# BananaFalls/LDPC-NeuralNetwork-Decoder

Hardware: AMD Instinct MI355X
Metric: codewords/s at fixed SNR (BG2, 10 iters) (higher is better)
Workload: dtype f32

## Files before the change

### ldpc-neuralnetwork-decoder_amd/csrc/flood_fixed.hpp

```cpp
#pragma once
#include "flood_host.hpp"
#include "gen/fixed_codes.hpp"

namespace ldpc {
namespace {

constexpr bool reg_edges(int algo) { return algo == LDPC_ALGO_MINSUM; }

#ifndef LDPC_SLOW_REG_EDGES
#define LDPC_SLOW_REG_EDGES 16
#endif
#ifndef LDPC_SLOW_REG_EDGES_OFF
#define LDPC_SLOW_REG_EDGES_OFF 6
#endif
constexpr int kAllRegEdges = 1 << 20;
template <int ES, bool BAIL>
constexpr int reg_edge_cap() {
    return BAIL ? kAllRegEdges : (ES == LDPC_ES_OFF ? LDPC_SLOW_REG_EDGES_OFF : LDPC_SLOW_REG_EDGES);
}

#ifndef LDPC_ROT_EDGES
#define LDPC_ROT_EDGES (1 << 20)
#endif
#ifndef LDPC_SLOW_ROT_EDGES
#define LDPC_SLOW_ROT_EDGES (1 << 20)
#endif
#ifndef LDPC_SLOW_ROT_EDGES_OFF
#define LDPC_SLOW_ROT_EDGES_OFF 0
#endif
template <int ES, bool BAIL>
constexpr int rot_edge_cap() {
    return BAIL ? LDPC_ROT_EDGES : (ES == LDPC_ES_OFF ? LDPC_SLOW_ROT_EDGES_OFF : LDPC_SLOW_ROT_EDGES);
}

template <class G, int WV, int CAP, int RCAP, bool REG>
struct FxPlan {
    static constexpr int R0 = REG ? G::RE_CHK_PTR[WV] : G::CHK_PTR[WV];
    static constexpr int NR = (REG ? G::RE_CHK_PTR[WV + 1] : G::CHK_PTR[WV + 1]) - R0;
    static constexpr int NREG = !REG ? 0 : (G::RE_NREG[WV] < CAP ? G::RE_NREG[WV] : CAP);
    static constexpr int chk_row(int i) { return REG ? G::RE_CHK_ROWS[R0 + i] : G::CHK_ROWS[R0 + i]; }
    static constexpr int row_shift(int e) { return REG ? G::RE_ROW_SHIFT[e] : G::ROW_SHIFT[e]; }
    static constexpr int col_shift(int j) { return REG ? G::RE_COL_SHIFT[j] : G::COL_SHIFT[j]; }
    static constexpr int row_reg(int e) { return REG && G::RE_ROW_REG[e] < CAP ? G::RE_ROW_REG[e] : -1; }
    static constexpr int col_reg(int j) { return REG && G::RE_COL_REG[j] < CAP ? G::RE_COL_REG[j] : -1; }
    static constexpr int col_slot_edges(int w) {
        int n = 0;
        for (int i = G::VT_COL_PTR[w]; i < G::VT_COL_PTR[w + 1]; ++i)
            for (int j = G::COL_PTR[G::VT_COLS[i]]; j < G::COL_PTR[G::VT_COLS[i] + 1]; ++j)
                if (G::COL_SLOT[j] >= 0 && G::RE_COL_REG[j] < 0) ++n;
        return n;
    }
    static constexpr int rot_share() {
        if (!REG) return 0;
        int left = RCAP;
        for (int w = 0; w < G::W; ++w) {
            const int a = col_slot_edges(w), b = col_slot_edges(WV);
            if (a > b || (a == b && w < WV)) left -= G::RE_NROT[w];
        }
        return left < 0 ? 0 : (left < G::RE_NROT[WV] ? left : G::RE_NROT[WV]);
    }
    static constexpr int NROT = rot_share();
    static constexpr int row_rot(int e) { return REG && G::RE_ROW_ROT[e] < NROT ? G::RE_ROW_ROT[e] : -1; }
    static constexpr int col_rot(int j) { return REG && G::RE_COL_ROT[j] < NROT ? G::RE_COL_ROT[j] : -1; }
    static constexpr int C0 = G::VT_COL_PTR[WV], NC = G::VT_COL_PTR[WV + 1] - C0;
    static constexpr int T0 = G::VT_PTR[WV], NT = G::VT_PTR[WV + 1] - T0;
    static constexpr int col_index(int col) {
        for (int i = 0; i < NC; ++i)
            if (G::VT_COLS[C0 + i] == col) return i;
        return -1;
    }
    struct Tab {
        int nsh = 0, next = 0, maxdc = 1, maxdv = 1;
        int shv[64] = {};
        int shidx[64] = {};
        int ext_before[64] = {};
    };
    static constexpr int inv_shift(int s) { return (G::Z - s) % G::Z; }
    static constexpr Tab make() {
        Tab t{};
        for (int i = 0; i < 64; ++i) t.shidx[i] = -1;
        auto use = [&t](int s) {
            if (t.shidx[s] < 0) {
                t.shidx[s] = t.nsh;
                t.shv[t.nsh++] = s;
            }
        };
        for (int i = 0; i < NC; ++i) {
            const int c = G::VT_COLS[C0 + i];
            const int dv = G::COL_PTR[c + 1] - G::COL_PTR[c];
            if (dv > t.maxdv) t.maxdv = dv;
            for (int j = G::COL_PTR[c]; j < G::COL_PTR[c + 1]; ++j)
                if (col_reg(j) < 0 && col_rot(j) < 0) use(col_shift(j));
        }
        for (int i = 0; i < NR; ++i) {
            const int R = chk_row(i);
            t.ext_before[i] = t.next;
            const int dc = G::ROW_PTR[R + 1] - G::ROW_PTR[R];
            if (dc > t.maxdc) t.maxdc = dc;
            for (int e = G::ROW_PTR[R]; e < G::ROW_PTR[R + 1]; ++e) {
                if (G::ROW_SLOT[e] < 0)
                    ++t.next;
                else if (row_reg(e) < 0 && row_rot(e) < 0)
                    use(inv_shift(row_shift(e)));
            }
        }
        return t;
    }
    static constexpr Tab T = make();
    static constexpr int ext_index(int i, int e) {
        const int R = chk_row(i);
        int x = T.ext_before[i];
        for (int q = 0; q < e; ++q)
            if (G::ROW_SLOT[G::ROW_PTR[R] + q] < 0) ++x;
        return x;
    }
};

constexpr int kVarPipe = 24;

#ifndef LDPC_DIRECT_DC
#define LDPC_DIRECT_DC 6
#endif
constexpr int kDirectDc = LDPC_DIRECT_DC;
static_assert(kDirectDc >= 0 && kDirectDc <= 6, "direct_row is written out for degrees 2 .. 6");

__device__ __forceinline__ uint32_t xor3(uint32_t a, uint32_t b, uint32_t c) { return __builtin_amdgcn_bitop3_b32(a, b, c, 0x96); }

template <int DC, int E, int CAP>
__device__ __forceinline__ float direct_row(const float (&v)[CAP], const float (&pr)[3], float als, float alv, uint32_t sgn) {
    static_assert(DC >= 2 && DC <= 6 && E < DC && DC <= CAP, "direct form: degrees 2 .. 6");
    constexpr int A = E == 0 ? 1 : 0, B = E <= 1 ? 2 : 1, Cc = E <= 2 ? 3 : 2;
    auto bits = [&](int e) { return __float_as_uint(v[e]); };
    if constexpr (DC == 2) {
        return __uint_as_float(__builtin_amdgcn_bitop3_b32(__float_as_uint(alv * fabsf(v[A])), bits(A), sgn, 0x78));
    } else if constexpr (DC == 3) {
        const float m = vmin(fabsf(v[A]), fabsf(v[B]));
        return __uint_as_float(__builtin_amdgcn_bitop3_b32(__float_as_uint(alv * m), bits(A) ^ bits(B), sgn, 0x78));
    } else if constexpr (DC == 4) {
        const float m = vmin(vmin(fabsf(v[A]), fabsf(v[B])), fabsf(v[Cc]));
        return __uint_as_float(__builtin_amdgcn_bitop3_b32(__float_as_uint(alv * m), xor3(bits(A), bits(B), bits(Cc)), sgn, 0x78));
    } else {
        constexpr int PE = E / 2;
        float m;
        if constexpr (DC == 5 && E == 4)
            m = vmin(pr[0], pr[1]);
        else if constexpr (DC == 5)
            m = vmin(vmin(fabsf(v[E ^ 1]), pr[1 - PE]), fabsf(v[4]));
        else
            m = vmin(vmin(fabsf(v[E ^ 1]), pr[(PE + 1) % 3]), pr[(PE + 2) % 3]);
        return __uint_as_float(__builtin_amdgcn_bitop3_b32(__float_as_uint(als * m), bits(E), sgn, 0x78));
    }
}

constexpr int kOutAny = 2;
template <class G, int OUT>
struct DecOut {
    static_assert(OUT == LDPC_OUT_U8 || OUT == LDPC_OUT_F32 || OUT == kOutAny, "one form per output type");
    static_assert(G::N % G::Z == 0 && (G::Z & (G::Z - 1)) == 0, "rotated(): row | position");
    char *base;
    uint32_t row;
    uint32_t own;
    uint32_t kb;
    uint32_t any;
    bool valid;
    __device__ __forceinline__ uint32_t size() const {
        if constexpr (OUT == kOutAny)
            return any;
        else
            return OUT == LDPC_OUT_F32 ? 4u : 1u;
    }
    __device__ __forceinline__ DecOut(const Ctx &C, const Lane &L) {
        any = C.out_dtype == LDPC_OUT_F32 ? 4u : 1u;
        base = static_cast<char *>(C.bits) + (int64_t)L.group * (64 / G::Z) * G::N * size();
        row = (uint32_t)L.f * (G::N * size());
        kb = (uint32_t)L.k * size();
        own = row + kb;
        valid = L.valid;
    }
    __device__ __forceinline__ void put(uint32_t off, int bit, int &errs) const {
        if (valid) {
            if (size() == 4u)
                *reinterpret_cast<float *>(base + off) = (float)bit;
            else
                *reinterpret_cast<uint8_t *>(base + off) = (uint8_t)bit;
        }
        errs += bit;
    }
    template <int COL>
    __device__ __forceinline__ void col(int bit, int &errs) const { put(own + COL * G::Z * size(), bit, errs); }
    template <int COL, int S>
    __device__ __forceinline__ void rotated(int bit, int &errs) const {
        put((row | ((kb + S * size()) & (G::Z * size() - 1))) + COL * G::Z * size(), bit, errs);
    }
};
struct NoOut {
    __device__ __forceinline__ NoOut(const Ctx &, const Lane &) {}
};
template <class G, int OUT>
using DecOutFor = std::conditional_t<OUT < 0, NoOut, DecOut<G, OUT>>;

template <class G, int ALGO, int WV, bool BAIL, int CAP, int RCAP, bool REG>
struct FixedBody {
    static_assert(!BAIL || ALGO == LDPC_ALGO_MINSUM, "only min-sum has a fast and an exact check update");
    static constexpr bool kBail = BAIL;
    static constexpr bool kPeel = true;
    using P = FxPlan<G, WV, CAP, RCAP, REG>;
    static constexpr int ZM4 = 4 * G::Z - 1;
    static constexpr int NEXT = P::T.next > 0 ? P::T.next : 1;
    static constexpr int NCOL = P::NC > 0 ? P::NC : 1;
    static constexpr int NSH = P::T.nsh > 0 ? P::T.nsh : 1;
    static constexpr int MAXDC = P::T.maxdc, MAXDV = P::T.maxdv;
    static constexpr int NRG = P::NREG > 0 ? P::NREG : 1;
    static constexpr int NRT = P::NROT > 0 ? P::NROT : 1;
    float ext[NEXT];
    float cllr[NCOL];
    uint32_t rot[NSH];
    float msg[NRG];
    float rmsg[NRT];


    template <int S>
    __device__ __forceinline__ float to_var_lane(float c2v) const { return seg_rotate<G::Z, S>(c2v); }
    template <int S>
    __device__ __forceinline__ float to_chk_lane(float v2c) const { return seg_rotate<G::Z, P::inv_shift(S)>(v2c); }

    __device__ __forceinline__ void init(Ctx &C, const Lane &L) {
        bool nan = false;
        sfor<P::NR>([&](auto i) {
            constexpr int I = decltype(i)::value, R = P::chk_row(I);
            constexpr int P0 = G::ROW_PTR[R], DC = G::ROW_PTR[R + 1] - P0;
            sfor<DC>([&](auto e) {
                constexpr int E = decltype(e)::value;
                if constexpr (G::ROW_SLOT[P0 + E] < 0) {
                    constexpr int X = P::ext_index(I, E), COL = G::ROW_COL[P0 + E], S4 = 4 * P::row_shift(P0 + E);
                    ext[X] = L.llr_at(COL * 4 * G::Z + ((L.k4 + S4) & ZM4));
                    nan |= !(fabsf(ext[X]) < INFINITY);
                }
            });
        });
        sfor<P::T.nsh>([&](auto j) {
            constexpr int J = decltype(j)::value, SH = P::T.shv[J];
            const uint32_t base = (uint32_t)(uintptr_t)C.lds;
            if constexpr (SH == 0)
                rot[J] = opaque_vu(base + L.lane4);
            else
                rot[J] = opaque_vu(base + L.fz4 + ((L.k4 + (4 * G::Z - 4 * SH)) & ZM4));
        });
        addtid_begin(C.lds);
        sfor<P::NC>([&](auto i) {
            constexpr int I = decltype(i)::value, COL = G::VT_COLS[P::C0 + I];
            constexpr int P0 = G::COL_PTR[COL], DV = G::COL_PTR[COL + 1] - P0;
            cllr[I] = L.llr_at(COL * 4 * G::Z + L.k4);
            nan |= !(fabsf(cllr[I]) < INFINITY);
            sfor<DV>([&](auto jj) {
                constexpr int J = P0 + decltype(jj)::value;
                if constexpr (P::col_reg(J) >= 0)
                    msg[P::col_reg(J)] = cllr[I];
                else if constexpr (P::col_rot(J) >= 0)
                    rmsg[P::col_rot(J)] = to_chk_lane<P::col_shift(J)>(cllr[I]);
                else
                    lds_wr_tid<G::COL_SLOT[J] * 256>(cllr[I]);
            });
        });
        addtid_end();
        if (__any(nan) && L.lane == 0) *C.flag = 1;
    }

    template <int I>
    __device__ __forceinline__ void load_row(const Ctx &C, const Lane &L, float (&v)[MAXDC]) const {
        constexpr int R = P::chk_row(I), P0 = G::ROW_PTR[R], DC = G::ROW_PTR[R + 1] - P0;
        sfor<DC>([&](auto e) {
            constexpr int E = decltype(e)::value, SL = G::ROW_SLOT[P0 + E];
            if constexpr (P::row_reg(P0 + E) >= 0)
                v[E] = msg[P::row_reg(P0 + E)];
            else if constexpr (P::row_rot(P0 + E) >= 0)
                v[E] = rmsg[P::row_rot(P0 + E)];
            else if constexpr (SL >= 0)
                v[E] = lds_rd_abs<SL * 256>(rot[P::T.shidx[P::inv_shift(P::row_shift(P0 + E))]]);
            else
                v[E] = ext[P::ext_index(I, E)];
        });
    }

    template <int I, bool DEC, bool SLOW, int OUT>
    __device__ __forceinline__ void row(const Ctx &C, const Lane &L, const DecOutFor<G, OUT> &D, const float (&v)[MAXDC], int &errs, float ninf, float pinf, uint32_t sgn, float alv) {
        constexpr int R = P::chk_row(I), P0 = G::ROW_PTR[R], DC = G::ROW_PTR[R + 1] - P0;
        auto needed = [](int e) constexpr { return DEC || G::ROW_SLOT[P0 + e] >= 0; };
        auto emit = [&](auto e, float o) {
            constexpr int E = decltype(e)::value, SL = G::ROW_SLOT[P0 + E];
            if constexpr (P::row_reg(P0 + E) >= 0) {
                msg[P::row_reg(P0 + E)] = o;
            } else if constexpr (P::row_rot(P0 + E) >= 0) {
                rmsg[P::row_rot(P0 + E)] = to_var_lane<P::row_shift(P0 + E)>(o);
            } else if constexpr (SL >= 0) {
                lds_wr_tid<SL * 256>(o);
            } else if constexpr (DEC) {
                constexpr int COL = G::ROW_COL[P0 + E], S = P::row_shift(P0 + E);
                const int bit = v[E] + o < 0.0f;
                if constexpr (OUT >= 0) D.template rotated<COL, S>(bit, errs);
                if (C.ballots) ext_ballot(C, L, COL, 4 * S, bit);
            }
        };
        if constexpr (ALGO == LDPC_ALGO_MINSUM && !SLOW && DC >= 2 && DC <= kDirectDc) {
            float pr[3] = {};
            float als = alv;
            if constexpr (DC >= 5) {
                sfor<DC / 2>([&](auto j) {
                    constexpr int J = decltype(j)::value;
                    pr[J] = vmin(fabsf(v[2 * J]), fabsf(v[2 * J + 1]));
                });
                uint32_t par = xor3(__float_as_uint(v[0]), __float_as_uint(v[1]), __float_as_uint(v[2]));
                if constexpr (DC == 5)
                    par = xor3(par, __float_as_uint(v[3]), __float_as_uint(v[4]));
                else
                    par = xor3(par, __float_as_uint(v[3]), __float_as_uint(v[4])) ^ __float_as_uint(v[5]);
                als = __uint_as_float(__builtin_amdgcn_bitop3_b32(__float_as_uint(alv), par, sgn, 0x78));
            }
            sfor<DC>([&](auto e) {
                constexpr int E = decltype(e)::value;
                if constexpr (needed(E)) emit(e, direct_row<DC, E>(v, pr, als, alv, sgn));
            });
        } else if constexpr (ALGO == LDPC_ALGO_MINSUM) {
            float m1 = fabsf(v[0]), m2 = pinf;
            two_smallest<DC>(v, m1, m2, ninf);
            if (!SLOW) {
                const uint32_t par = sign_parity_n<DC>(v) & sgn;
                const uint32_t s1 = __float_as_uint(alv * m1) ^ par, s2 = __float_as_uint(alv * m2) ^ par;
                uint64_t mk[DC];
                uint32_t sel[DC];
                sfor<DC + 3>([&](auto q) {
                    constexpr int Q = decltype(q)::value;
                    if constexpr (Q < DC && needed(Q)) mk[Q] = cmp_eq_abs(v[Q], m1);
                    if constexpr (Q >= 3 && needed(Q - 3)) sel[Q - 3] = cndmask(s1, s2, mk[Q - 3]);
                });
                sfor<DC>([&](auto e) {
                    constexpr int E = decltype(e)::value;
                    if constexpr (needed(E))
                        emit(e, __uint_as_float(__builtin_amdgcn_bitop3_b32(sel[E], __float_as_uint(v[E]), sgn, 0x78)));
                });
            } else {
                MinSumStats st;
                sfor<DC>([&](auto e) { st.add(decltype(e)::value, v[decltype(e)::value]); });
                sfor<DC>([&](auto e) { emit(e, st.c2v(decltype(e)::value, v[decltype(e)::value], C.alpha)); });
            }
        } else {
            float acc[DC];
            float Pp = 1.0f;
            sfor<DC>([&](auto jj) {
                constexpr int J = decltype(jj)::value;
                const float t = tanh_half(v[J]);
                sfor<J>([&](auto e) { acc[decltype(e)::value] = acc[decltype(e)::value] * t; });
                acc[J] = Pp;
                Pp = Pp * t;
            });
            sfor<DC>([&](auto e) { emit(e, two_atanh(acc[decltype(e)::value])); });
        }
    }

    template <bool DEC, bool DIRECT>
    __device__ __forceinline__ void check(const Ctx &C, const Lane &L, int &errs) {
        static_assert(DEC || !DIRECT, "stores need decisions");
        if constexpr (ALGO == LDPC_ALGO_MINSUM && !BAIL) {
            if (__builtin_amdgcn_readfirstlane(*C.flag) != 0) {
                rows<DEC, true, (DIRECT ? kOutAny : -1)>(C, L, errs);
                return;
            }
        }
        if constexpr (!DIRECT)
            rows<DEC, false, -1>(C, L, errs);
        else if (C.out_dtype == LDPC_OUT_F32)
            rows<DEC, false, LDPC_OUT_F32>(C, L, errs);
        else
            rows<DEC, false, LDPC_OUT_U8>(C, L, errs);
    }

    template <bool DEC, bool SLOW, int OUT>
    __device__ __forceinline__ void rows(const Ctx &C, const Lane &L, int &errs) {
        float va[MAXDC], vb[MAXDC];
        const DecOutFor<G, OUT> D(C, L);
        addtid_begin(C.lds);
        const float ninf = opaque_sf(-INFINITY), pinf = opaque_sf(INFINITY);
        const uint32_t sgn = opaque_vu(0x80000000u);
        const float alv = opaque_vf(C.alpha);
        load_row<0>(C, L, va);
        sfor<P::NR>([&](auto i) {
            constexpr int I = decltype(i)::value;
            if constexpr (I % 2 == 0) {
                if constexpr (I + 1 < P::NR) load_row<I + 1>(C, L, vb);
                row<I, DEC, SLOW, OUT>(C, L, D, va, errs, ninf, pinf, sgn, alv);
            } else {
                if constexpr (I + 1 < P::NR) load_row<I + 1>(C, L, va);
                row<I, DEC, SLOW, OUT>(C, L, D, vb, errs, ninf, pinf, sgn, alv);
            }
        });
        addtid_end();
    }

    template <int TK>
    struct Task {
        static constexpr int X = P::T0 + TK;
        static constexpr int CA = G::VT_A[X], CB = G::VT_B[X];
        static constexpr int PA = G::COL_PTR[CA], DA = G::COL_PTR[CA + 1] - PA;
        static constexpr int PB = CB >= 0 ? G::COL_PTR[CB] : 0, DB = CB >= 0 ? G::COL_PTR[CB + 1] - PB : 0;
        static_assert(DB <= DA, "pair tasks: A is the longer column");
        static constexpr int IA = P::col_index(CA), IB = CB >= 0 ? P::col_index(CB) : 0;
        static constexpr int NMSG = DA + DB;
    };
    struct TaskIn {
        f32x2 cp[MAXDV];
        float cs[MAXDV];
    };

    template <int X>
    __device__ __forceinline__ float c2v_in() const {
        if constexpr (P::col_reg(X) >= 0)
            return msg[P::col_reg(X)];
        else if constexpr (P::col_rot(X) >= 0)
            return rmsg[P::col_rot(X)];
        else
            return lds_rd_abs<G::COL_SLOT[X] * 256>(rot[P::T.shidx[P::col_shift(X)]]);
    }
    template <int X>
    __device__ __forceinline__ void v2c_out(float o) {
        if constexpr (P::col_reg(X) >= 0)
            msg[P::col_reg(X)] = o;
        else if constexpr (P::col_rot(X) >= 0)
            rmsg[P::col_rot(X)] = to_chk_lane<P::col_shift(X)>(o);
        else
            lds_wr_tid<G::COL_SLOT[X] * 256>(o);
    }

    template <int TK>
    __device__ __forceinline__ void load_task(const Ctx &C, TaskIn &in) const {
        using K = Task<TK>;
        sfor<K::DA>([&](auto jj) {
            constexpr int J = decltype(jj)::value;
            if constexpr (J < K::DB) {
                in.cp[J].x = c2v_in<K::PA + J>();
                in.cp[J].y = c2v_in<K::PB + J>();
            } else {
                in.cs[J] = c2v_in<K::PA + J>();
            }
        });
    }

    template <int TK, bool DEC, bool WRITE, int OUT>
    __device__ __forceinline__ void task(const Ctx &C, const Lane &L, const DecOutFor<G, OUT> &D, const TaskIn &in, int &errs, bool &bad) {
        using K = Task<TK>;
        constexpr int DA = K::DA, DB = K::DB;
        f32x2 P2;
        float PA = cllr[K::IA];
        if constexpr (DB > 0) {
            P2.x = cllr[K::IA];
            P2.y = cllr[K::IB];
        }
        f32x2 acc2[DB > 0 ? DB : 1];
        float accA[DA];
        sfor<DA>([&](auto jj) {
            constexpr int J = decltype(jj)::value;
            if constexpr (J < DB) {
                sfor<J>([&](auto e) {
                    constexpr int E = decltype(e)::value;
                    acc2[E] = acc2[E] + in.cp[J];
                });
                acc2[J] = P2;
                P2 = P2 + in.cp[J];
                if constexpr (J == DB - 1) PA = P2.x;
            } else {
                sfor<J>([&](auto e) {
                    constexpr int E = decltype(e)::value;
                    if constexpr (E < DB)
                        acc2[E].x = acc2[E].x + in.cs[J];
                    else
                        accA[E] = accA[E] + in.cs[J];
                });
                accA[J] = PA;
                PA = PA + in.cs[J];
            }
        });
        if constexpr (WRITE) {
            sfor<DA>([&](auto e) {
                constexpr int E = decltype(e)::value;
                if constexpr (E < DB) {
                    v2c_out<K::PA + E>(acc2[E].x);
                    v2c_out<K::PB + E>(acc2[E].y);
                } else {
                    v2c_out<K::PA + E>(accA[E]);
                }
            });
        }
        auto decide = [&](auto col, float app) {
            constexpr int COL = decltype(col)::value;
            const int bit = app < 0.0f;
            if constexpr (OUT >= 0) D.template col<COL>(bit, errs);
            if (C.ballots) var_ballot(C, L, COL, bit);
        };
        if constexpr (ALGO == LDPC_ALGO_MINSUM) bad |= !(fabsf(PA) < INFINITY);
        if constexpr (DEC) decide(ic<K::CA>{}, PA);
        if constexpr (DB > 0) {
            if constexpr (ALGO == LDPC_ALGO_MINSUM) bad |= !(fabsf(P2.y) < INFINITY);
            if constexpr (DEC) decide(ic<K::CB>{}, P2.y);
        }
    }

    template <bool DEC, bool WRITE, bool DIRECT>
    __device__ __forceinline__ void var(const Ctx &C, const Lane &L, int &errs) {
        static_assert(DEC || !DIRECT, "stores need decisions");
        if constexpr (!DIRECT)
            var_as<DEC, WRITE, -1>(C, L, errs);
        else if (C.out_dtype == LDPC_OUT_F32)
            var_as<DEC, WRITE, LDPC_OUT_F32>(C, L, errs);
        else
            var_as<DEC, WRITE, LDPC_OUT_U8>(C, L, errs);
    }
    template <bool DEC, bool WRITE, int OUT>
    __device__ __forceinline__ void var_as(const Ctx &C, const Lane &L, int &errs) {
        bool bad = false;
        if constexpr (P::NT > 0) {
            const DecOutFor<G, OUT> D(C, L);
            TaskIn ta, tb;
            if constexpr (WRITE) addtid_begin(C.lds);
            load_task<0>(C, ta);
            sfor<P::NT>([&](auto i) {
                constexpr int I = decltype(i)::value;
                constexpr bool more = I + 1 < P::NT;
                constexpr bool ahead = more && Task<I>::NMSG + Task<(more ? I + 1 : I)>::NMSG <= kVarPipe;
                if constexpr (I % 2 == 0) {
                    if constexpr (ahead) load_task<I + 1>(C, tb);
                    task<I, DEC, WRITE, OUT>(C, L, D, ta, errs, bad);
                    if constexpr (more && !ahead) load_task<(more ? I + 1 : I)>(C, tb);
                } else {
                    if constexpr (ahead) load_task<I + 1>(C, ta);
                    task<I, DEC, WRITE, OUT>(C, L, D, tb, errs, bad);
                    if constexpr (more && !ahead) load_task<(more ? I + 1 : I)>(C, ta);
                }
            });
            if constexpr (WRITE) addtid_end();
        }
        if constexpr (ALGO == LDPC_ALGO_MINSUM) {
            if (__any(bad) && L.lane == 0) *C.flag = 1;
        }
    }

    __device__ __forceinline__ int parity(const Ctx &C, const Lane &L) const {
        int inv = 0;
        int f = L.f, k = L.k;
        asm volatile("" : "+v"(f), "+v"(k));
        sfor<P::NR>([&](auto i) {
            constexpr int R = P::chk_row(decltype(i)::value);
            constexpr int P0 = G::ROW_PTR[R], DC = G::ROW_PTR[R + 1] - P0;
            int p = 0;
            sfor<DC>([&](auto e) {
                constexpr int E = decltype(e)::value;
                constexpr int COL = G::ROW_COL[P0 + E], S = P::row_shift(P0 + E);
                p ^= (int)(C.words[COL] >> (f * G::Z + ((k + S) & (G::Z - 1))));
            });
            inv |= p;
        });
        return inv & 1;
    }
};

template <class G, class F>
__device__ __forceinline__ void fx_by_wave(int wave, F &&f) {
    static_assert(G::W == 4, "fixed schedules are generated for 4 waves");
    switch (wave) {
        case 0: f(ic<0>{}); break;
        case 1: f(ic<1>{}); break;
        case 2: f(ic<2>{}); break;
        default: f(ic<3>{}); break;
    }
}

}

template <class G, int ALGO, int ES, bool BAIL = false>
__global__ __launch_bounds__(256, ES == LDPC_ES_OFF ? 4 : 3) void flood_fixed_kernel(FloodTables T, const float *__restrict__ llr,
                                                          int64_t B, int max_iter, float alpha, int out_dtype,
                                                          void *__restrict__ bits, Outs O, EsWs W, uint32_t *redo) {
    static_assert(!BAIL || ES == LDPC_ES_OFF || ES == LDPC_ES_FRAME, "the batch-stop passes share state across workgroups");
    extern __shared__ __attribute__((aligned(16))) char lds[];
#ifdef LDPC_TIMELINE
    const uint64_t t_in = tl_now();
#endif
    FloodTables Tc = T;
    Tc.Z = G::Z, Tc.FG = 64 / G::Z, Tc.Mb = G::Mb, Tc.Nb = G::Nb, Tc.N = G::N, Tc.nslots = G::NSLOTS, Tc.W = G::W;
    static_assert(G::Z < 64 && 64 % G::Z == 0, "rep1 below: a 1 at the bottom of every Z-bit segment");
    Tc.rep1 = ~0ull / ((1ull << G::Z) - 1ull);
    const Lane L = make_lane(Tc, llr, B);
    Ctx C;
    init_ctx(C, Tc, lds, alpha, out_dtype, bits);
    if constexpr (BAIL) C.redo = redo;
    fx_by_wave<G>(__builtin_amdgcn_readfirstlane((int)threadIdx.x >> 6), [&](auto wv) {
        FixedBody<G, ALGO, decltype(wv)::value, BAIL, reg_edge_cap<ES, BAIL>(), rot_edge_cap<ES, BAIL>(), reg_edges(ALGO)> body;
        flood_drive<ES>(body, C, L, B, max_iter, O, W);
#ifdef LDPC_TIMELINE
        if constexpr (ES == LDPC_ES_OFF) tl_bracket(O.timeline, decltype(wv)::value, t_in);
#endif
    });
}

template <int ALGO>
int launch_fixed(const FloodCall &c, int es, size_t lds, const Outs &O, const EsWs &W, uint32_t *redo) {
    auto pick = [&](auto code) -> const void * {
        using G = decltype(code);
        if constexpr (ALGO == LDPC_ALGO_MINSUM) {
            if (redo && es == LDPC_ES_OFF) return reinterpret_cast<const void *>(flood_fixed_kernel<G, ALGO, LDPC_ES_OFF, true>);
            if (redo && es == LDPC_ES_FRAME) return reinterpret_cast<const void *>(flood_fixed_kernel<G, ALGO, LDPC_ES_FRAME, true>);
        }
        if (redo) return nullptr;
        switch (es) {
            case LDPC_ES_OFF: return reinterpret_cast<const void *>(flood_fixed_kernel<G, ALGO, LDPC_ES_OFF>);
            case LDPC_ES_FRAME: return reinterpret_cast<const void *>(flood_fixed_kernel<G, ALGO, LDPC_ES_FRAME>);
            case LDPC_ES_BATCH: return reinterpret_cast<const void *>(flood_fixed_kernel<G, ALGO, LDPC_ES_BATCH>);
            case ES_P1: return reinterpret_cast<const void *>(flood_fixed_kernel<G, ALGO, ES_P1>);
            case ES_P2: return reinterpret_cast<const void *>(flood_fixed_kernel<G, ALGO, ES_P2>);
            default: return nullptr;
        }
    };
    const int id = c.g->fixed_id;
    const void *kern = id == 1 ? pick(fixed::BG2_Z4{}) : (id == 2 ? pick(fixed::BG2_Z32{}) : nullptr);
    if (!kern) return fail(LDPC_EINVAL, "no fixed kernel for this code / stopping mode");
    LDPC_HIP(hipFuncSetAttribute(kern, hipFuncAttributeMaxDynamicSharedMemorySize, (int)lds));
    FloodCall a = c;
    FloodTables t = c.g->ft;
    Outs o = O;
    EsWs w = W;
    void *args[] = {&t, &a.llr, &a.B, &a.max_iter, &a.alpha, &a.out_dtype, &a.bits, &o, &w, &redo};
    const int64_t nwg = (c.B + c.g->FG - 1) / c.g->FG;
    LDPC_HIP(hipLaunchKernel(kern, dim3((unsigned)nwg), dim3(64 * c.g->ft.W), args, lds, c.s));
    return LDPC_OK;
}

}
```

### ldpc-neuralnetwork-decoder_amd/csrc/gen/fixed_codes.hpp

```cpp
#pragma once

namespace ldpc {
namespace fixed {

struct BG2_Z4 {
    static constexpr int Z = 4, Mb = 42, Nb = 52, N = 208, NSLOTS = 159, W = 4;
    static constexpr int NBLOCKS = 197;
    static constexpr int BLK_ROW[197] = {0, 0, 0, 0, 0, 0, 0, 0, 1, 1, 1, 1, 1, 1, 1, 1, 1, 1, 2, 2, 2, 2, 2, 2, 2, 2, 3, 3, 3, 3, 3, 3, 3, 3, 3, 3, 4, 4, 4, 4, 5, 5, 5, 5, 5, 5, 6, 6, 6, 6, 6, 6, 7, 7, 7, 7, 7, 7, 8, 8, 8, 8, 9, 9, 9, 9, 9, 10, 10, 10, 10, 10, 11, 11, 11, 11, 11, 12, 12, 12, 12, 13, 13, 13, 13, 13, 14, 14, 14, 14, 14, 15, 15, 15, 15, 16, 16, 16, 16, 16, 17, 17, 17, 17, 17, 18, 18, 18, 18, 19, 19, 19, 19, 20, 20, 20, 20, 21, 21, 21, 21, 22, 22, 22, 23, 23, 23, 23, 24, 24, 24, 24, 25, 25, 25, 26, 26, 26, 26, 26, 27, 27, 27, 28, 28, 28, 28, 29, 29, 29, 30, 30, 30, 30, 30, 31, 31, 31, 32, 32, 32, 32, 33, 33, 33, 33, 34, 34, 34, 34, 35, 35, 35, 35, 36, 36, 36, 36, 37, 37, 37, 38, 38, 38, 38, 39, 39, 39, 39, 40, 40, 40, 40, 41, 41, 41, 41};
    static constexpr int BLK_COL[197] = {0, 1, 2, 3, 6, 9, 10, 11, 0, 3, 4, 5, 6, 7, 8, 9, 11, 12, 0, 1, 3, 4, 8, 10, 12, 13, 1, 2, 4, 5, 6, 7, 8, 9, 10, 13, 0, 1, 11, 14, 0, 1, 5, 7, 11, 15, 0, 5, 7, 9, 11, 16, 1, 5, 7, 11, 13, 17, 0, 1, 12, 18, 1, 8, 10, 11, 19, 0, 1, 6, 7, 20, 0, 7, 9, 13, 21, 1, 3, 11, 22, 0, 1, 8, 13, 23, 1, 6, 11, 13, 24, 0, 10, 11, 25, 1, 9, 11, 12, 26, 1, 5, 11, 12, 27, 0, 6, 7, 28, 0, 1, 10, 29, 1, 4, 11, 30, 0, 8, 13, 31, 1, 2, 32, 0, 3, 5, 33, 1, 2, 9, 34, 0, 5, 35, 2, 7, 12, 13, 36, 0, 6, 37, 1, 2, 5, 38, 0, 4, 39, 2, 5, 7, 9, 40, 1, 13, 41, 0, 5, 12, 42, 2, 7, 10, 43, 0, 12, 13, 44, 1, 5, 11, 45, 0, 2, 7, 46, 10, 13, 47, 1, 5, 11, 48, 0, 7, 12, 49, 2, 10, 13, 50, 1, 5, 11, 51};
    static constexpr int BLK_SHIFT[197] = {1, 1, 0, 2, 1, 1, 0, 0, 3, 2, 1, 1, 2, 0, 0, 0, 0, 0, 1, 2, 0, 0, 0, 1, 0, 0, 0, 2, 2, 0, 1, 2, 2, 0, 0, 0, 3, 2, 3, 0, 3, 1, 2, 3, 3, 0, 3, 0, 1, 0, 2, 0, 1, 3, 0, 3, 0, 0, 2, 2, 2, 0, 3, 1, 1, 3, 0, 3, 1, 0, 1, 0, 3, 0, 2, 0, 0, 3, 3, 2, 0, 3, 2, 2, 2, 0, 3, 1, 3, 0, 0, 3, 3, 1, 0, 3, 2, 0, 2, 0, 2, 0, 2, 0, 0, 0, 2, 2, 0, 3, 0, 1, 0, 2, 1, 1, 0, 0, 2, 2, 0, 2, 3, 0, 3, 3, 2, 0, 2, 3, 0, 0, 0, 0, 0, 1, 3, 0, 2, 0, 0, 3, 0, 2, 1, 3, 0, 2, 0, 0, 3, 0, 1, 0, 0, 2, 1, 0, 2, 0, 2, 0, 0, 0, 3, 0, 3, 1, 0, 0, 1, 0, 3, 0, 0, 2, 2, 0, 3, 3, 0, 3, 2, 2, 0, 3, 0, 2, 0, 0, 3, 0, 0, 1, 1, 2, 0};
    static constexpr int ROW_PTR[43] = {0, 8, 18, 26, 36, 40, 46, 52, 58, 62, 67, 72, 77, 81, 86, 91, 95, 100, 105, 109, 113, 117, 121, 124, 128, 132, 135, 140, 143, 147, 150, 155, 158, 162, 166, 170, 174, 178, 181, 185, 189, 193, 197};
    static constexpr int ROW_SLOT[197] = {0, 1, 2, 3, 4, 5, 6, 7, 8, 9, 10, 11, 12, 13, 14, 15, 16, 17, 18, 19, 20, 21, 22, 23, 24, 25, 26, 27, 28, 29, 30, 31, 32, 33, 34, 35, 36, 37, 38, -1, 39, 40, 41, 42, 43, -1, 44, 45, 46, 47, 48, -1, 49, 50, 51, 52, 53, -1, 54, 55, 56, -1, 57, 58, 59, 60, -1, 61, 62, 63, 64, -1, 65, 66, 67, 68, -1, 69, 70, 71, -1, 72, 73, 74, 75, -1, 76, 77, 78, 79, -1, 80, 81, 82, -1, 83, 84, 85, 86, -1, 87, 88, 89, 90, -1, 91, 92, 93, -1, 94, 95, 96, -1, 97, 98, 99, -1, 100, 101, 102, -1, 103, 104, -1, 105, 106, 107, -1, 108, 109, 110, -1, 111, 112, -1, 113, 114, 115, 116, -1, 117, 118, -1, 119, 120, 121, -1, 122, 123, -1, 124, 125, 126, 127, -1, 128, 129, -1, 130, 131, 132, -1, 133, 134, 135, -1, 136, 137, 138, -1, 139, 140, 141, -1, 142, 143, 144, -1, 145, 146, -1, 147, 148, 149, -1, 150, 151, 152, -1, 153, 154, 155, -1, 156, 157, 158, -1};
    static constexpr int ROW_COL[197] = {0, 1, 2, 3, 6, 9, 10, 11, 0, 3, 4, 5, 6, 7, 8, 9, 11, 12, 0, 1, 3, 4, 8, 10, 12, 13, 1, 2, 4, 5, 6, 7, 8, 9, 10, 13, 0, 1, 11, 14, 0, 1, 5, 7, 11, 15, 0, 5, 7, 9, 11, 16, 1, 5, 7, 11, 13, 17, 0, 1, 12, 18, 1, 8, 10, 11, 19, 0, 1, 6, 7, 20, 0, 7, 9, 13, 21, 1, 3, 11, 22, 0, 1, 8, 13, 23, 1, 6, 11, 13, 24, 0, 10, 11, 25, 1, 9, 11, 12, 26, 1, 5, 11, 12, 27, 0, 6, 7, 28, 0, 1, 10, 29, 1, 4, 11, 30, 0, 8, 13, 31, 1, 2, 32, 0, 3, 5, 33, 1, 2, 9, 34, 0, 5, 35, 2, 7, 12, 13, 36, 0, 6, 37, 1, 2, 5, 38, 0, 4, 39, 2, 5, 7, 9, 40, 1, 13, 41, 0, 5, 12, 42, 2, 7, 10, 43, 0, 12, 13, 44, 1, 5, 11, 45, 0, 2, 7, 46, 10, 13, 47, 1, 5, 11, 48, 0, 7, 12, 49, 2, 10, 13, 50, 1, 5, 11, 51};
    static constexpr int ROW_SHIFT[197] = {1, 1, 0, 2, 1, 1, 0, 0, 3, 2, 1, 1, 2, 0, 0, 0, 0, 0, 1, 2, 0, 0, 0, 1, 0, 0, 0, 2, 2, 0, 1, 2, 2, 0, 0, 0, 3, 2, 3, 0, 3, 1, 2, 3, 3, 0, 3, 0, 1, 0, 2, 0, 1, 3, 0, 3, 0, 0, 2, 2, 2, 0, 3, 1, 1, 3, 0, 3, 1, 0, 1, 0, 3, 0, 2, 0, 0, 3, 3, 2, 0, 3, 2, 2, 2, 0, 3, 1, 3, 0, 0, 3, 3, 1, 0, 3, 2, 0, 2, 0, 2, 0, 2, 0, 0, 0, 2, 2, 0, 3, 0, 1, 0, 2, 1, 1, 0, 0, 2, 2, 0, 2, 3, 0, 3, 3, 2, 0, 2, 3, 0, 0, 0, 0, 0, 1, 3, 0, 2, 0, 0, 3, 0, 2, 1, 3, 0, 2, 0, 0, 3, 0, 1, 0, 0, 2, 1, 0, 2, 0, 2, 0, 0, 0, 3, 0, 3, 1, 0, 0, 1, 0, 3, 0, 0, 2, 2, 0, 3, 3, 0, 3, 2, 2, 0, 3, 0, 2, 0, 0, 3, 0, 0, 1, 1, 2, 0};
    static constexpr int COL_PTR[53] = {0, 22, 45, 55, 60, 65, 79, 86, 99, 105, 113, 122, 138, 147, 159, 160, 161, 162, 163, 164, 165, 166, 167, 168, 169, 170, 171, 172, 173, 174, 175, 176, 177, 178, 179, 180, 181, 182, 183, 184, 185, 186, 187, 188, 189, 190, 191, 192, 193, 194, 195, 196, 197};
    static constexpr int COL_SLOT[197] = {0, 8, 18, 36, 39, 44, 54, 61, 65, 72, 80, 91, 94, 100, 105, 111, 117, 122, 130, 136, 142, 150, 1, 19, 26, 37, 40, 49, 55, 57, 62, 69, 73, 76, 83, 87, 95, 97, 103, 108, 119, 128, 139, 147, 156, 2, 27, 104, 109, 113, 120, 124, 133, 143, 153, 3, 9, 20, 70, 106, 10, 21, 28, 98, 123, 11, 29, 41, 45, 50, 88, 107, 112, 121, 125, 131, 140, 148, 157, 4, 12, 30, 63, 77, 92, 118, 13, 31, 42, 46, 51, 64, 66, 93, 114, 126, 134, 144, 151, 14, 22, 32, 58, 74, 101, 5, 15, 33, 47, 67, 84, 110, 127, 6, 23, 34, 59, 81, 96, 135, 145, 154, 7, 16, 38, 43, 48, 52, 60, 71, 78, 82, 85, 89, 99, 141, 149, 158, 17, 24, 56, 86, 90, 115, 132, 137, 152, 25, 35, 53, 68, 75, 79, 102, 116, 129, 138, 146, 155, -1, -1, -1, -1, -1, -1, -1, -1, -1, -1, -1, -1, -1, -1, -1, -1, -1, -1, -1, -1, -1, -1, -1, -1, -1, -1, -1, -1, -1, -1, -1, -1, -1, -1, -1, -1, -1, -1};
    static constexpr int COL_SHIFT[197] = {1, 3, 1, 3, 3, 3, 2, 3, 3, 3, 3, 0, 3, 0, 3, 0, 0, 2, 2, 3, 0, 3, 1, 2, 0, 2, 1, 1, 2, 3, 1, 3, 2, 3, 3, 2, 0, 2, 2, 2, 2, 2, 1, 3, 1, 0, 2, 3, 3, 1, 1, 3, 0, 2, 0, 2, 2, 0, 3, 3, 1, 0, 2, 1, 0, 1, 0, 2, 0, 3, 0, 2, 0, 3, 0, 0, 0, 2, 1, 1, 2, 1, 0, 1, 2, 3, 0, 2, 3, 1, 0, 1, 0, 2, 3, 1, 0, 2, 0, 0, 0, 2, 1, 2, 2, 1, 0, 0, 0, 2, 2, 0, 0, 0, 1, 0, 1, 3, 1, 3, 3, 3, 0, 0, 3, 3, 2, 3, 3, 2, 3, 1, 0, 2, 1, 3, 2, 2, 0, 0, 2, 2, 0, 0, 2, 1, 2, 0, 0, 0, 0, 2, 0, 2, 2, 1, 0, 3, 0, 0, 0, 0, 0, 0, 0, 0, 0, 0, 0, 0, 0, 0, 0, 0, 0, 0, 0, 0, 0, 0, 0, 0, 0, 0, 0, 0, 0, 0, 0, 0, 0, 0, 0, 0, 0, 0, 0};
    static constexpr int CHK_PTR[5] = {0, 10, 21, 32, 42};
    static constexpr int CHK_ROWS[42] = {3, 9, 12, 13, 15, 20, 26, 28, 35, 40, 0, 4, 5, 10, 16, 18, 22, 23, 29, 33, 38, 2, 6, 8, 11, 17, 19, 24, 25, 31, 34, 39, 1, 7, 14, 21, 27, 30, 32, 36, 37, 41};
    static constexpr int VT_COL_PTR[5] = {0, 3, 7, 10, 14};
    static constexpr int VT_COLS[14] = {0, 4, 12, 3, 5, 9, 11, 1, 6, 8, 2, 7, 10, 13};
    static constexpr int VT_PTR[5] = {0, 3, 6, 8, 10};
    static constexpr int VT_A[10] = {0, 4, 12, 3, 9, 11, 1, 6, 2, 7};
    static constexpr int VT_B[10] = {-1, -1, -1, -1, -1, 5, -1, 8, 10, 13};
    static constexpr int BW_PTR[5] = {0, 13, 26, 39, 52};
    static constexpr int BW_COLS[52] = {0, 4, 8, 12, 16, 20, 24, 28, 32, 36, 40, 44, 48, 1, 5, 9, 13, 17, 21, 25, 29, 33, 37, 41, 45, 49, 2, 6, 10, 14, 18, 22, 26, 30, 34, 38, 42, 46, 50, 3, 7, 11, 15, 19, 23, 27, 31, 35, 39, 43, 47, 51};
    static constexpr int RE_CAP = 16;
    static constexpr int RE_RHO[42] = {3, 0, 0, 0, 1, 1, 0, 1, 2, 3, 0, 0, 1, 2, 1, 1, 2, 2, 0, 0, 2, 0, 2, 1, 2, 0, 1, 1, 1, 0, 0, 2, 2, 0, 1, 0, 2, 1, 2, 1, 0, 3};
    static constexpr int RE_ROW_SHIFT[197] = {0, 0, 3, 1, 0, 0, 3, 3, 3, 2, 1, 1, 2, 0, 0, 0, 0, 0, 1, 2, 0, 0, 0, 1, 0, 0, 0, 2, 2, 0, 1, 2, 2, 0, 0, 0, 0, 3, 0, 1, 0, 2, 3, 0, 0, 1, 3, 0, 1, 0, 2, 0, 2, 0, 1, 0, 1, 1, 0, 0, 0, 2, 2, 0, 0, 2, 3, 3, 1, 0, 1, 0, 3, 0, 2, 0, 0, 0, 0, 3, 1, 1, 0, 0, 0, 2, 0, 2, 0, 1, 1, 0, 0, 2, 1, 1, 0, 2, 0, 2, 0, 2, 0, 2, 2, 0, 2, 2, 0, 3, 0, 1, 0, 0, 3, 3, 2, 0, 2, 2, 0, 0, 1, 2, 0, 0, 3, 1, 0, 1, 2, 2, 0, 0, 0, 2, 0, 1, 3, 1, 1, 0, 1, 3, 2, 0, 1, 2, 0, 0, 3, 0, 1, 0, 0, 0, 3, 2, 0, 2, 0, 2, 0, 0, 3, 0, 0, 2, 1, 1, 1, 0, 3, 0, 2, 0, 0, 2, 0, 0, 1, 1, 0, 0, 2, 0, 1, 3, 1, 0, 3, 0, 0, 0, 0, 1, 3};
    static constexpr int RE_COL_SHIFT[197] = {0, 3, 1, 0, 0, 3, 0, 3, 3, 1, 0, 0, 3, 0, 0, 0, 1, 2, 0, 0, 2, 0, 0, 2, 0, 3, 2, 2, 0, 2, 1, 0, 0, 0, 1, 0, 0, 0, 0, 0, 3, 0, 1, 1, 0, 3, 2, 1, 1, 2, 2, 3, 0, 0, 0, 1, 2, 0, 0, 0, 1, 0, 2, 3, 0, 1, 0, 3, 0, 0, 2, 3, 0, 0, 0, 2, 0, 0, 0, 0, 2, 1, 0, 2, 2, 0, 0, 2, 0, 1, 1, 1, 0, 2, 0, 1, 0, 0, 1, 0, 0, 2, 0, 0, 2, 0, 0, 0, 0, 2, 0, 2, 0, 3, 1, 0, 0, 0, 1, 3, 0, 3, 3, 0, 0, 0, 2, 0, 2, 3, 0, 2, 2, 0, 3, 3, 0, 1, 0, 0, 0, 0, 2, 1, 0, 2, 3, 0, 0, 1, 0, 0, 1, 2, 3, 3, 1, 0, 0, 1, 1, 0, 1, 2, 3, 0, 0, 1, 2, 1, 1, 2, 2, 0, 0, 2, 0, 2, 1, 2, 0, 1, 1, 1, 0, 0, 2, 2, 0, 1, 0, 2, 1, 2, 1, 0, 3};
    static constexpr int RE_ROW_REG[197] = {-1, 0, -1, -1, 1, -1, -1, -1, -1, -1, -1, -1, -1, -1, -1, 0, 1, -1, -1, -1, -1, 0, -1, -1, 1, -1, -1, -1, -1, -1, -1, -1, -1, -1, 0, 1, 2, -1, -1, -1, -1, -1, -1, 2, -1, -1, -1, 2, -1, 3, -1, -1, -1, 4, -1, 5, -1, -1, 3, -1, 4, -1, -1, -1, 3, -1, -1, -1, -1, 2, -1, -1, -1, 4, -1, 5, -1, 3, -1, -1, -1, -1, 4, 5, -1, -1, -1, -1, 6, -1, -1, 5, -1, -1, -1, -1, -1, -1, 6, -1, 6, -1, -1, -1, -1, 7, -1, -1, -1, -1, 7, -1, -1, 8, -1, -1, -1, 8, -1, -1, -1, 9, -1, -1, 9, -1, -1, -1, 10, -1, -1, -1, -1, 7, -1, -1, 6, -1, -1, -1, -1, 11, -1, -1, -1, 8, -1, -1, 10, -1, -1, 9, -1, 10, -1, 12, -1, -1, 11, -1, 12, -1, 7, 8, -1, -1, 13, -1, -1, -1, -1, 11, -1, -1, -1, 9, 10, -1, 11, 12, -1, -1, 12, 13, -1, 14, -1, -1, -1, 13, -1, 14, -1, 13, -1, -1, -1};
    static constexpr int RE_COL_REG[197] = {-1, -1, -1, 2, -1, -1, 3, -1, -1, -1, 5, 7, -1, 8, 9, -1, -1, -1, 11, 13, -1, 14, 0, -1, -1, -1, -1, -1, -1, -1, -1, 3, 4, -1, -1, 6, 7, 8, 9, 10, -1, 12, -1, -1, 13, -1, -1, -1, -1, -1, -1, -1, 7, 9, 13, -1, -1, -1, -1, -1, -1, 0, -1, -1, 10, -1, -1, -1, 2, 4, -1, -1, 7, 8, 9, -1, 11, 12, -1, 1, -1, -1, 2, -1, -1, 11, -1, -1, 2, -1, -1, -1, 4, -1, 6, -1, 8, 10, -1, -1, -1, -1, -1, 5, -1, -1, 0, -1, 3, -1, -1, -1, 10, -1, -1, 0, 3, -1, -1, -1, 11, -1, -1, 1, -1, -1, -1, 5, -1, -1, 6, -1, -1, -1, -1, -1, 13, -1, -1, 1, 4, 6, -1, -1, 12, -1, -1, -1, 1, -1, 5, -1, -1, -1, -1, -1, -1, 12, 14, -1, -1, -1, -1, -1, -1, -1, -1, -1, -1, -1, -1, -1, -1, -1, -1, -1, -1, -1, -1, -1, -1, -1, -1, -1, -1, -1, -1, -1, -1, -1, -1, -1, -1, -1, -1, -1, -1};
    static constexpr int RE_NREG[4] = {15, 14, 14, 15};
    static constexpr int RE_CHK_PTR[5] = {0, 12, 21, 33, 42};
    static constexpr int RE_CHK_ROWS[42] = {2, 4, 8, 15, 16, 18, 21, 23, 29, 32, 34, 39, 1, 6, 7, 14, 25, 28, 30, 35, 38, 0, 10, 12, 13, 17, 19, 20, 22, 24, 27, 31, 41, 3, 5, 9, 11, 26, 33, 36, 37, 40};
    static constexpr int RE_ROW_ROT[197] = {-1, -1, -1, -1, -1, -1, -1, -1, -1, 0, -1, 1, -1, -1, -1, -1, -1, -1, 0, -1, -1, -1, -1, -1, -1, -1, -1, 0, -1, -1, -1, 1, -1, -1, -1, -1, -1, -1, -1, -1, -1, -1, -1, -1, -1, -1, -1, -1, -1, -1, 2, -1, -1, -1, -1, -1, -1, -1, -1, -1, -1, -1, -1, -1, -1, -1, -1, -1, 0, -1, -1, -1, -1, -1, -1, -1, -1, -1, -1, -1, -1, -1, -1, -1, -1, -1, -1, -1, -1, -1, -1, -1, -1, -1, -1, -1, -1, -1, -1, -1, -1, -1, -1, -1, -1, -1, -1, -1, -1, -1, -1, -1, -1, -1, -1, -1, -1, -1, -1, -1, -1, -1, -1, -1, -1, -1, -1, -1, -1, -1, -1, -1, -1, -1, -1, 2, -1, -1, 3, -1, -1, -1, -1, -1, -1, -1, -1, 1, -1, -1, -1, -1, -1, -1, -1, -1, -1, -1, -1, -1, -1, -1, -1, -1, 4, -1, -1, 2, -1, -1, -1, -1, 3, -1, -1, -1, -1, -1, -1, -1, -1, -1, -1, -1, -1, -1, -1, 3, -1, -1, 5, -1, -1, -1, -1, -1, -1};
    static constexpr int RE_COL_ROT[197] = {-1, -1, 0, -1, -1, -1, -1, -1, -1, -1, -1, -1, -1, -1, -1, -1, -1, 1, -1, -1, -1, -1, -1, -1, -1, -1, -1, -1, -1, -1, 0, -1, -1, -1, -1, -1, -1, -1, -1, -1, -1, -1, -1, -1, -1, -1, 0, -1, -1, 2, -1, -1, -1, -1, -1, -1, 0, -1, -1, -1, -1, -1, -1, -1, -1, 1, -1, -1, -1, -1, -1, -1, -1, -1, -1, -1, -1, -1, -1, -1, -1, -1, -1, -1, -1, -1, -1, 1, -1, -1, -1, -1, -1, -1, -1, -1, -1, -1, -1, -1, -1, -1, -1, -1, -1, -1, -1, -1, -1, -1, -1, -1, -1, -1, -1, -1, -1, -1, -1, 4, -1, 5, -1, -1, -1, -1, 2, -1, -1, -1, -1, -1, -1, -1, -1, 3, -1, -1, -1, -1, -1, -1, -1, -1, -1, 2, 3, -1, -1, -1, -1, -1, -1, -1, 3, -1, -1, -1, -1, -1, -1, -1, -1, -1, -1, -1, -1, -1, -1, -1, -1, -1, -1, -1, -1, -1, -1, -1, -1, -1, -1, -1, -1, -1, -1, -1, -1, -1, -1, -1, -1, -1, -1, -1, -1, -1, -1};
    static constexpr int RE_NROT[4] = {4, 4, 1, 6};
};

struct BG2_Z32 {
    static constexpr int Z = 32, Mb = 42, Nb = 52, N = 1664, NSLOTS = 159, W = 4;
    static constexpr int NBLOCKS = 197;
    static constexpr int BLK_ROW[197] = {0, 0, 0, 0, 0, 0, 0, 0, 1, 1, 1, 1, 1, 1, 1, 1, 1, 1, 2, 2, 2, 2, 2, 2, 2, 2, 3, 3, 3, 3, 3, 3, 3, 3, 3, 3, 4, 4, 4, 4, 5, 5, 5, 5, 5, 5, 6, 6, 6, 6, 6, 6, 7, 7, 7, 7, 7, 7, 8, 8, 8, 8, 9, 9, 9, 9, 9, 10, 10, 10, 10, 10, 11, 11, 11, 11, 11, 12, 12, 12, 12, 13, 13, 13, 13, 13, 14, 14, 14, 14, 14, 15, 15, 15, 15, 16, 16, 16, 16, 16, 17, 17, 17, 17, 17, 18, 18, 18, 18, 19, 19, 19, 19, 20, 20, 20, 20, 21, 21, 21, 21, 22, 22, 22, 23, 23, 23, 23, 24, 24, 24, 24, 25, 25, 25, 26, 26, 26, 26, 26, 27, 27, 27, 28, 28, 28, 28, 29, 29, 29, 30, 30, 30, 30, 30, 31, 31, 31, 32, 32, 32, 32, 33, 33, 33, 33, 34, 34, 34, 34, 35, 35, 35, 35, 36, 36, 36, 36, 37, 37, 37, 38, 38, 38, 38, 39, 39, 39, 39, 40, 40, 40, 40, 41, 41, 41, 41};
    static constexpr int BLK_COL[197] = {0, 1, 2, 3, 6, 9, 10, 11, 0, 3, 4, 5, 6, 7, 8, 9, 11, 12, 0, 1, 3, 4, 8, 10, 12, 13, 1, 2, 4, 5, 6, 7, 8, 9, 10, 13, 0, 1, 11, 14, 0, 1, 5, 7, 11, 15, 0, 5, 7, 9, 11, 16, 1, 5, 7, 11, 13, 17, 0, 1, 12, 18, 1, 8, 10, 11, 19, 0, 1, 6, 7, 20, 0, 7, 9, 13, 21, 1, 3, 11, 22, 0, 1, 8, 13, 23, 1, 6, 11, 13, 24, 0, 10, 11, 25, 1, 9, 11, 12, 26, 1, 5, 11, 12, 27, 0, 6, 7, 28, 0, 1, 10, 29, 1, 4, 11, 30, 0, 8, 13, 31, 1, 2, 32, 0, 3, 5, 33, 1, 2, 9, 34, 0, 5, 35, 2, 7, 12, 13, 36, 0, 6, 37, 1, 2, 5, 38, 0, 4, 39, 2, 5, 7, 9, 40, 1, 13, 41, 0, 5, 12, 42, 2, 7, 10, 43, 0, 12, 13, 44, 1, 5, 11, 45, 0, 2, 7, 46, 10, 13, 47, 1, 5, 11, 48, 0, 7, 12, 49, 2, 10, 13, 50, 1, 5, 11, 51};
    static constexpr int BLK_SHIFT[197] = {9, 21, 12, 26, 29, 13, 0, 0, 7, 6, 29, 29, 2, 28, 0, 28, 0, 0, 17, 18, 12, 20, 16, 1, 0, 0, 8, 26, 30, 8, 17, 22, 18, 0, 0, 0, 19, 22, 7, 0, 7, 9, 2, 31, 7, 0, 27, 4, 13, 28, 30, 0, 1, 19, 12, 3, 20, 0, 14, 30, 6, 0, 11, 13, 29, 23, 0, 11, 25, 0, 21, 0, 11, 12, 18, 24, 0, 31, 15, 14, 0, 19, 2, 6, 30, 0, 19, 17, 3, 8, 0, 19, 15, 21, 0, 11, 14, 8, 18, 0, 30, 28, 18, 0, 0, 28, 2, 18, 0, 23, 20, 25, 0, 26, 9, 29, 0, 12, 10, 18, 0, 30, 31, 0, 23, 11, 14, 0, 14, 11, 8, 0, 4, 28, 0, 29, 15, 0, 26, 0, 8, 23, 0, 2, 5, 7, 0, 18, 28, 0, 7, 16, 9, 20, 0, 10, 1, 0, 18, 12, 6, 0, 4, 4, 11, 0, 19, 21, 4, 0, 25, 8, 31, 0, 12, 6, 26, 0, 27, 23, 0, 31, 2, 6, 0, 15, 12, 2, 0, 0, 11, 24, 0, 1, 5, 22, 0};
    static constexpr int ROW_PTR[43] = {0, 8, 18, 26, 36, 40, 46, 52, 58, 62, 67, 72, 77, 81, 86, 91, 95, 100, 105, 109, 113, 117, 121, 124, 128, 132, 135, 140, 143, 147, 150, 155, 158, 162, 166, 170, 174, 178, 181, 185, 189, 193, 197};
    static constexpr int ROW_SLOT[197] = {0, 1, 2, 3, 4, 5, 6, 7, 8, 9, 10, 11, 12, 13, 14, 15, 16, 17, 18, 19, 20, 21, 22, 23, 24, 25, 26, 27, 28, 29, 30, 31, 32, 33, 34, 35, 36, 37, 38, -1, 39, 40, 41, 42, 43, -1, 44, 45, 46, 47, 48, -1, 49, 50, 51, 52, 53, -1, 54, 55, 56, -1, 57, 58, 59, 60, -1, 61, 62, 63, 64, -1, 65, 66, 67, 68, -1, 69, 70, 71, -1, 72, 73, 74, 75, -1, 76, 77, 78, 79, -1, 80, 81, 82, -1, 83, 84, 85, 86, -1, 87, 88, 89, 90, -1, 91, 92, 93, -1, 94, 95, 96, -1, 97, 98, 99, -1, 100, 101, 102, -1, 103, 104, -1, 105, 106, 107, -1, 108, 109, 110, -1, 111, 112, -1, 113, 114, 115, 116, -1, 117, 118, -1, 119, 120, 121, -1, 122, 123, -1, 124, 125, 126, 127, -1, 128, 129, -1, 130, 131, 132, -1, 133, 134, 135, -1, 136, 137, 138, -1, 139, 140, 141, -1, 142, 143, 144, -1, 145, 146, -1, 147, 148, 149, -1, 150, 151, 152, -1, 153, 154, 155, -1, 156, 157, 158, -1};
    static constexpr int ROW_COL[197] = {0, 1, 2, 3, 6, 9, 10, 11, 0, 3, 4, 5, 6, 7, 8, 9, 11, 12, 0, 1, 3, 4, 8, 10, 12, 13, 1, 2, 4, 5, 6, 7, 8, 9, 10, 13, 0, 1, 11, 14, 0, 1, 5, 7, 11, 15, 0, 5, 7, 9, 11, 16, 1, 5, 7, 11, 13, 17, 0, 1, 12, 18, 1, 8, 10, 11, 19, 0, 1, 6, 7, 20, 0, 7, 9, 13, 21, 1, 3, 11, 22, 0, 1, 8, 13, 23, 1, 6, 11, 13, 24, 0, 10, 11, 25, 1, 9, 11, 12, 26, 1, 5, 11, 12, 27, 0, 6, 7, 28, 0, 1, 10, 29, 1, 4, 11, 30, 0, 8, 13, 31, 1, 2, 32, 0, 3, 5, 33, 1, 2, 9, 34, 0, 5, 35, 2, 7, 12, 13, 36, 0, 6, 37, 1, 2, 5, 38, 0, 4, 39, 2, 5, 7, 9, 40, 1, 13, 41, 0, 5, 12, 42, 2, 7, 10, 43, 0, 12, 13, 44, 1, 5, 11, 45, 0, 2, 7, 46, 10, 13, 47, 1, 5, 11, 48, 0, 7, 12, 49, 2, 10, 13, 50, 1, 5, 11, 51};
    static constexpr int ROW_SHIFT[197] = {9, 21, 12, 26, 29, 13, 0, 0, 7, 6, 29, 29, 2, 28, 0, 28, 0, 0, 17, 18, 12, 20, 16, 1, 0, 0, 8, 26, 30, 8, 17, 22, 18, 0, 0, 0, 19, 22, 7, 0, 7, 9, 2, 31, 7, 0, 27, 4, 13, 28, 30, 0, 1, 19, 12, 3, 20, 0, 14, 30, 6, 0, 11, 13, 29, 23, 0, 11, 25, 0, 21, 0, 11, 12, 18, 24, 0, 31, 15, 14, 0, 19, 2, 6, 30, 0, 19, 17, 3, 8, 0, 19, 15, 21, 0, 11, 14, 8, 18, 0, 30, 28, 18, 0, 0, 28, 2, 18, 0, 23, 20, 25, 0, 26, 9, 29, 0, 12, 10, 18, 0, 30, 31, 0, 23, 11, 14, 0, 14, 11, 8, 0, 4, 28, 0, 29, 15, 0, 26, 0, 8, 23, 0, 2, 5, 7, 0, 18, 28, 0, 7, 16, 9, 20, 0, 10, 1, 0, 18, 12, 6, 0, 4, 4, 11, 0, 19, 21, 4, 0, 25, 8, 31, 0, 12, 6, 26, 0, 27, 23, 0, 31, 2, 6, 0, 15, 12, 2, 0, 0, 11, 24, 0, 1, 5, 22, 0};
    static constexpr int COL_PTR[53] = {0, 22, 45, 55, 60, 65, 79, 86, 99, 105, 113, 122, 138, 147, 159, 160, 161, 162, 163, 164, 165, 166, 167, 168, 169, 170, 171, 172, 173, 174, 175, 176, 177, 178, 179, 180, 181, 182, 183, 184, 185, 186, 187, 188, 189, 190, 191, 192, 193, 194, 195, 196, 197};
    static constexpr int COL_SLOT[197] = {0, 8, 18, 36, 39, 44, 54, 61, 65, 72, 80, 91, 94, 100, 105, 111, 117, 122, 130, 136, 142, 150, 1, 19, 26, 37, 40, 49, 55, 57, 62, 69, 73, 76, 83, 87, 95, 97, 103, 108, 119, 128, 139, 147, 156, 2, 27, 104, 109, 113, 120, 124, 133, 143, 153, 3, 9, 20, 70, 106, 10, 21, 28, 98, 123, 11, 29, 41, 45, 50, 88, 107, 112, 121, 125, 131, 140, 148, 157, 4, 12, 30, 63, 77, 92, 118, 13, 31, 42, 46, 51, 64, 66, 93, 114, 126, 134, 144, 151, 14, 22, 32, 58, 74, 101, 5, 15, 33, 47, 67, 84, 110, 127, 6, 23, 34, 59, 81, 96, 135, 145, 154, 7, 16, 38, 43, 48, 52, 60, 71, 78, 82, 85, 89, 99, 141, 149, 158, 17, 24, 56, 86, 90, 115, 132, 137, 152, 25, 35, 53, 68, 75, 79, 102, 116, 129, 138, 146, 155, -1, -1, -1, -1, -1, -1, -1, -1, -1, -1, -1, -1, -1, -1, -1, -1, -1, -1, -1, -1, -1, -1, -1, -1, -1, -1, -1, -1, -1, -1, -1, -1, -1, -1, -1, -1, -1, -1};
    static constexpr int COL_SHIFT[197] = {9, 7, 17, 19, 7, 27, 14, 11, 11, 19, 19, 28, 23, 12, 23, 4, 8, 18, 18, 19, 12, 15, 21, 18, 8, 22, 9, 1, 30, 11, 25, 31, 2, 19, 11, 30, 20, 26, 30, 14, 2, 10, 25, 31, 1, 12, 26, 31, 11, 29, 5, 7, 4, 6, 0, 26, 6, 12, 15, 11, 29, 20, 30, 9, 28, 29, 8, 2, 4, 19, 28, 14, 28, 7, 16, 12, 8, 2, 5, 29, 2, 17, 0, 17, 2, 23, 28, 22, 31, 13, 12, 21, 12, 18, 15, 9, 4, 26, 12, 0, 16, 18, 13, 6, 10, 13, 28, 0, 28, 18, 14, 8, 20, 0, 1, 0, 29, 15, 25, 11, 27, 11, 0, 0, 7, 7, 30, 3, 23, 14, 3, 21, 8, 18, 29, 31, 6, 22, 0, 0, 6, 18, 0, 0, 6, 21, 2, 0, 0, 20, 24, 30, 8, 18, 26, 1, 4, 23, 24, 0, 0, 0, 0, 0, 0, 0, 0, 0, 0, 0, 0, 0, 0, 0, 0, 0, 0, 0, 0, 0, 0, 0, 0, 0, 0, 0, 0, 0, 0, 0, 0, 0, 0, 0, 0, 0, 0};
    static constexpr int CHK_PTR[5] = {0, 10, 21, 32, 42};
    static constexpr int CHK_ROWS[42] = {3, 9, 12, 13, 15, 20, 26, 28, 35, 40, 0, 4, 5, 10, 16, 18, 22, 23, 29, 33, 38, 2, 6, 8, 11, 17, 19, 24, 25, 31, 34, 39, 1, 7, 14, 21, 27, 30, 32, 36, 37, 41};
    static constexpr int VT_COL_PTR[5] = {0, 3, 7, 10, 14};
    static constexpr int VT_COLS[14] = {0, 4, 12, 3, 5, 9, 11, 1, 6, 8, 2, 7, 10, 13};
    static constexpr int VT_PTR[5] = {0, 3, 6, 8, 10};
    static constexpr int VT_A[10] = {0, 4, 12, 3, 9, 11, 1, 6, 2, 7};
    static constexpr int VT_B[10] = {-1, -1, -1, -1, -1, 5, -1, 8, 10, 13};
    static constexpr int BW_PTR[5] = {0, 13, 26, 39, 52};
    static constexpr int BW_COLS[52] = {0, 4, 8, 12, 16, 20, 24, 28, 32, 36, 40, 44, 48, 1, 5, 9, 13, 17, 21, 25, 29, 33, 37, 41, 45, 49, 2, 6, 10, 14, 18, 22, 26, 30, 34, 38, 42, 46, 50, 3, 7, 11, 15, 19, 23, 27, 31, 35, 39, 43, 47, 51};
    static constexpr int RE_CAP = 16;
    static constexpr int RE_RHO[42] = {6, 0, 14, 0, 13, 1, 19, 31, 2, 21, 11, 14, 1, 2, 13, 11, 18, 0, 4, 9, 3, 20, 2, 21, 18, 4, 0, 24, 30, 4, 12, 22, 20, 28, 11, 7, 20, 5, 30, 20, 0, 10};
    static constexpr int RE_ROW_SHIFT[197] = {15, 27, 18, 0, 3, 19, 6, 6, 7, 6, 29, 29, 2, 28, 0, 28, 0, 0, 31, 0, 26, 2, 30, 15, 14, 14, 8, 26, 30, 8, 17, 22, 18, 0, 0, 0, 0, 3, 20, 13, 8, 10, 3, 0, 8, 1, 14, 23, 0, 15, 17, 19, 0, 18, 11, 2, 19, 31, 16, 0, 8, 2, 0, 2, 18, 12, 21, 22, 4, 11, 0, 11, 25, 26, 0, 6, 14, 0, 16, 15, 1, 21, 4, 8, 0, 2, 0, 30, 16, 21, 13, 30, 26, 0, 11, 29, 0, 26, 4, 18, 30, 28, 18, 0, 0, 0, 6, 22, 4, 0, 29, 2, 9, 29, 12, 0, 3, 0, 30, 6, 20, 0, 1, 2, 12, 0, 3, 21, 0, 29, 26, 18, 8, 0, 4, 29, 15, 0, 26, 0, 0, 15, 24, 0, 3, 5, 30, 22, 0, 4, 19, 28, 21, 0, 12, 0, 23, 22, 6, 0, 26, 20, 0, 0, 7, 28, 30, 0, 15, 11, 0, 15, 6, 7, 0, 26, 14, 20, 0, 28, 5, 29, 0, 4, 30, 3, 0, 22, 20, 0, 11, 24, 0, 11, 15, 0, 10};
    static constexpr int RE_COL_SHIFT[197] = {15, 7, 31, 0, 8, 14, 16, 22, 25, 21, 30, 0, 0, 0, 12, 8, 0, 22, 6, 30, 0, 3, 27, 0, 8, 3, 10, 0, 0, 0, 4, 0, 4, 0, 29, 30, 29, 29, 0, 0, 0, 0, 0, 29, 11, 18, 26, 1, 29, 29, 3, 19, 0, 26, 0, 0, 6, 26, 16, 0, 29, 2, 30, 12, 0, 29, 8, 3, 23, 18, 28, 3, 0, 5, 28, 0, 15, 0, 15, 3, 2, 17, 11, 30, 6, 15, 28, 22, 0, 0, 11, 0, 26, 22, 15, 21, 0, 14, 0, 0, 30, 18, 2, 8, 30, 19, 28, 0, 15, 0, 0, 26, 0, 6, 15, 0, 18, 26, 2, 7, 0, 11, 6, 0, 20, 8, 17, 2, 12, 15, 16, 0, 26, 18, 0, 6, 4, 0, 0, 14, 8, 4, 0, 0, 26, 0, 22, 14, 0, 19, 6, 0, 21, 6, 26, 23, 15, 28, 24, 13, 1, 19, 31, 2, 21, 11, 14, 1, 2, 13, 11, 18, 0, 4, 9, 3, 20, 2, 21, 18, 4, 0, 24, 30, 4, 12, 22, 20, 28, 11, 7, 20, 5, 30, 20, 0, 10};
    static constexpr int RE_ROW_REG[197] = {-1, -1, -1, 0, -1, -1, -1, -1, -1, -1, -1, -1, -1, -1, -1, -1, -1, 0, -1, 0, -1, -1, -1, -1, -1, -1, -1, -1, -1, -1, -1, -1, -1, -1, 0, 1, 1, -1, -1, -1, -1, -1, -1, 2, -1, -1, -1, -1, 3, -1, -1, -1, 1, -1, -1, -1, -1, -1, -1, 2, -1, -1, 3, -1, -1, -1, -1, -1, -1, -1, 4, -1, -1, -1, 1, -1, -1, 4, -1, -1, -1, -1, -1, -1, 5, -1, 5, -1, -1, -1, -1, -1, -1, 2, -1, -1, 3, -1, -1, -1, -1, -1, -1, 2, -1, 3, -1, -1, -1, 4, -1, -1, -1, -1, -1, 4, -1, 5, -1, -1, -1, 6, -1, -1, -1, 5, -1, -1, 7, -1, -1, -1, -1, 6, -1, -1, -1, 6, -1, -1, 7, -1, -1, 8, -1, -1, -1, -1, 8, -1, -1, -1, -1, 7, -1, 9, -1, -1, -1, 8, -1, -1, 6, 7, -1, -1, -1, 9, -1, -1, 10, -1, -1, -1, 10, -1, -1, -1, 8, -1, -1, -1, 9, -1, -1, -1, 9, -1, -1, 10, -1, -1, -1, -1, -1, 10, -1};
    static constexpr int RE_COL_REG[197] = {-1, -1, -1, 1, -1, -1, -1, -1, -1, -1, -1, 3, 4, 5, -1, -1, 7, -1, -1, -1, 10, -1, -1, 0, -1, -1, -1, 1, 2, 3, -1, 4, -1, 5, -1, -1, -1, -1, 6, 7, 8, 9, 10, -1, -1, -1, -1, -1, -1, -1, -1, -1, 6, -1, 10, 0, -1, -1, -1, 5, -1, -1, -1, -1, 8, -1, -1, -1, -1, -1, -1, -1, 6, -1, -1, 8, -1, 9, -1, -1, -1, -1, -1, -1, -1, -1, -1, -1, 2, 3, -1, 4, -1, -1, -1, -1, 7, -1, 9, -1, -1, -1, -1, -1, -1, -1, -1, -1, -1, 1, 3, -1, 7, -1, -1, 0, -1, -1, -1, -1, 8, -1, -1, -1, -1, -1, -1, -1, -1, -1, -1, 2, -1, -1, 4, -1, -1, 10, 0, -1, -1, -1, 2, 6, -1, 9, -1, -1, 1, -1, -1, 5, -1, -1, -1, -1, -1, -1, -1, -1, -1, -1, -1, -1, -1, -1, -1, -1, -1, -1, -1, -1, -1, -1, -1, -1, -1, -1, -1, -1, -1, -1, -1, -1, -1, -1, -1, -1, -1, -1, -1, -1, -1, -1, -1, -1, -1};
    static constexpr int RE_NREG[4] = {11, 11, 11, 11};
    static constexpr int RE_CHK_PTR[5] = {0, 11, 22, 33, 42};
    static constexpr int RE_CHK_ROWS[42] = {1, 4, 17, 18, 19, 21, 26, 27, 29, 34, 36, 0, 11, 15, 16, 20, 23, 25, 30, 32, 38, 41, 2, 7, 8, 9, 12, 14, 22, 24, 28, 31, 35, 3, 5, 6, 10, 13, 33, 37, 39, 40};
    static constexpr int RE_ROW_ROT[197] = {-1, -1, -1, -1, -1, 0, -1, 1, 0, -1, 1, -1, -1, -1, -1, -1, -1, -1, -1, -1, -1, -1, 0, -1, -1, -1, -1, 0, -1, -1, -1, 1, -1, -1, -1, -1, -1, -1, -1, -1, -1, -1, -1, -1, -1, -1, -1, -1, -1, -1, -1, -1, -1, -1, -1, -1, -1, -1, -1, -1, -1, -1, -1, 1, -1, -1, -1, -1, -1, -1, -1, -1, -1, -1, -1, -1, -1, -1, -1, -1, -1, -1, -1, -1, -1, -1, -1, 2, -1, -1, -1, -1, -1, -1, -1, -1, -1, 2, -1, -1, -1, -1, -1, -1, -1, -1, -1, -1, -1, -1, -1, -1, -1, -1, -1, -1, -1, -1, -1, -1, -1, -1, -1, -1, -1, -1, 3, -1, -1, -1, -1, -1, -1, -1, -1, -1, -1, -1, -1, -1, -1, -1, -1, -1, -1, -1, -1, 2, -1, -1, -1, 4, -1, -1, -1, -1, -1, -1, -1, -1, -1, -1, -1, -1, 2, -1, 3, -1, -1, -1, -1, -1, -1, -1, -1, -1, -1, -1, -1, 3, -1, -1, -1, 5, -1, -1, -1, -1, -1, -1, 4, 5, -1, -1, 6, -1, -1};
    static constexpr int RE_COL_ROT[197] = {-1, 0, -1, -1, -1, -1, -1, -1, -1, -1, -1, -1, -1, -1, -1, -1, -1, 2, -1, 3, -1, -1, -1, -1, -1, -1, -1, -1, -1, -1, -1, -1, -1, -1, -1, -1, -1, -1, -1, -1, -1, -1, -1, -1, -1, -1, 0, -1, -1, -1, -1, -1, -1, -1, -1, -1, -1, -1, -1, -1, 1, -1, -1, -1, -1, -1, -1, -1, -1, -1, -1, 3, -1, -1, 4, -1, -1, -1, 6, -1, -1, -1, -1, 2, -1, -1, -1, 1, -1, -1, -1, -1, -1, -1, -1, -1, -1, -1, -1, -1, 0, -1, 1, -1, -1, 0, -1, -1, -1, -1, -1, -1, -1, -1, -1, -1, -1, -1, -1, 2, -1, 4, 1, -1, -1, -1, -1, -1, -1, -1, -1, -1, 2, -1, -1, -1, 5, -1, -1, -1, -1, -1, -1, -1, -1, -1, -1, -1, -1, -1, -1, -1, -1, -1, -1, -1, -1, 3, 5, -1, -1, -1, -1, -1, -1, -1, -1, -1, -1, -1, -1, -1, -1, -1, -1, -1, -1, -1, -1, -1, -1, -1, -1, -1, -1, -1, -1, -1, -1, -1, -1, -1, -1, -1, -1, -1, -1};
    static constexpr int RE_NROT[4] = {4, 7, 3, 6};
};

}
}
```

Baseline: 75.97 million.

## Add joint check/variable wave partition schedule for register-edge min-sum decoding

Adds a second, jointly optimized assignment of check rows and variable columns to waves, together with the per-code tables for it: row lifting, register-edge and rotation-edge slots, and column/task lists. The plan struct now reads the joint tables whenever the joint family flag is set; by default that covers the bail and non-bail min-sum variants with early stopping on, plus bail with it off. The goal is to keep more edge messages in registers or rotations and fewer in LDS, and to balance the check and variable work across waves. In exchange, register pressure rises (larger NREG/NROT) and there is one extra cllr slot.

```diff
diff --git a/ldpc-neuralnetwork-decoder_amd/csrc/flood_fixed.hpp b/ldpc-neuralnetwork-decoder_amd/csrc/flood_fixed.hpp
--- a/ldpc-neuralnetwork-decoder_amd/csrc/flood_fixed.hpp
+++ b/ldpc-neuralnetwork-decoder_amd/csrc/flood_fixed.hpp
@@ -33,21 +33,45 @@
     return BAIL ? LDPC_ROT_EDGES : (ES == LDPC_ES_OFF ? LDPC_SLOW_ROT_EDGES_OFF : LDPC_SLOW_ROT_EDGES);
 }
 
-template <class G, int WV, int CAP, int RCAP, bool REG>
+#ifndef LDPC_JOINT_MASK
+#define LDPC_JOINT_MASK 11
+#endif
+template <class G, int ALGO, int ES, bool BAIL>
+constexpr bool joint_family() {
+    if (!reg_edges(ALGO)) return false;
+    const int bit = BAIL ? (ES == LDPC_ES_OFF ? 0 : 1) : (ES == LDPC_ES_OFF ? 2 : 3);
+    return (LDPC_JOINT_MASK >> bit) & 1;
+}
+
+template <class G, int WV, int CAP, int RCAP, bool REG, bool JOINT>
 struct FxPlan {
-    static constexpr int R0 = REG ? G::RE_CHK_PTR[WV] : G::CHK_PTR[WV];
-    static constexpr int NR = (REG ? G::RE_CHK_PTR[WV + 1] : G::CHK_PTR[WV + 1]) - R0;
-    static constexpr int NREG = !REG ? 0 : (G::RE_NREG[WV] < CAP ? G::RE_NREG[WV] : CAP);
-    static constexpr int chk_row(int i) { return REG ? G::RE_CHK_ROWS[R0 + i] : G::CHK_ROWS[R0 + i]; }
-    static constexpr int row_shift(int e) { return REG ? G::RE_ROW_SHIFT[e] : G::ROW_SHIFT[e]; }
-    static constexpr int col_shift(int j) { return REG ? G::RE_COL_SHIFT[j] : G::COL_SHIFT[j]; }
-    static constexpr int row_reg(int e) { return REG && G::RE_ROW_REG[e] < CAP ? G::RE_ROW_REG[e] : -1; }
-    static constexpr int col_reg(int j) { return REG && G::RE_COL_REG[j] < CAP ? G::RE_COL_REG[j] : -1; }
+    static_assert(REG || !JOINT, "the joint schedule is a register-edge schedule");
+    static constexpr int chk_ptr(int w) { return JOINT ? G::RE_J_CHK_PTR[w] : (REG ? G::RE_CHK_PTR[w] : G::CHK_PTR[w]); }
+    static constexpr int chk_rows(int x) { return JOINT ? G::RE_J_CHK_ROWS[x] : (REG ? G::RE_CHK_ROWS[x] : G::CHK_ROWS[x]); }
+    static constexpr int nreg(int w) { return JOINT ? G::RE_J_NREG[w] : G::RE_NREG[w]; }
+    static constexpr int nrot(int w) { return JOINT ? G::RE_J_NROT[w] : G::RE_NROT[w]; }
+    static constexpr int row_reg_all(int e) { return JOINT ? G::RE_J_ROW_REG[e] : G::RE_ROW_REG[e]; }
+    static constexpr int col_reg_all(int j) { return JOINT ? G::RE_J_COL_REG[j] : G::RE_COL_REG[j]; }
+    static constexpr int row_rot_all(int e) { return JOINT ? G::RE_J_ROW_ROT[e] : G::RE_ROW_ROT[e]; }
+    static constexpr int col_rot_all(int j) { return JOINT ? G::RE_J_COL_ROT[j] : G::RE_COL_ROT[j]; }
+    static constexpr int vt_col_ptr(int w) { return JOINT ? G::RE_J_VT_COL_PTR[w] : G::VT_COL_PTR[w]; }
+    static constexpr int vt_cols(int x) { return JOINT ? G::RE_J_VT_COLS[x] : G::VT_COLS[x]; }
+    static constexpr int vt_ptr(int w) { return JOINT ? G::RE_J_VT_PTR[w] : G::VT_PTR[w]; }
+    static constexpr int vt_a(int x) { return JOINT ? G::RE_J_VT_A[x] : G::VT_A[x]; }
+    static constexpr int vt_b(int x) { return JOINT ? G::RE_J_VT_B[x] : G::VT_B[x]; }
+    static constexpr int R0 = chk_ptr(WV);
+    static constexpr int NR = chk_ptr(WV + 1) - R0;
+    static constexpr int NREG = !REG ? 0 : (nreg(WV) < CAP ? nreg(WV) : CAP);
+    static constexpr int chk_row(int i) { return chk_rows(R0 + i); }
+    static constexpr int row_shift(int e) { return JOINT ? G::RE_J_ROW_SHIFT[e] : (REG ? G::RE_ROW_SHIFT[e] : G::ROW_SHIFT[e]); }
+    static constexpr int col_shift(int j) { return JOINT ? G::RE_J_COL_SHIFT[j] : (REG ? G::RE_COL_SHIFT[j] : G::COL_SHIFT[j]); }
+    static constexpr int row_reg(int e) { return REG && row_reg_all(e) < CAP ? row_reg_all(e) : -1; }
+    static constexpr int col_reg(int j) { return REG && col_reg_all(j) < CAP ? col_reg_all(j) : -1; }
     static constexpr int col_slot_edges(int w) {
         int n = 0;
-        for (int i = G::VT_COL_PTR[w]; i < G::VT_COL_PTR[w + 1]; ++i)
-            for (int j = G::COL_PTR[G::VT_COLS[i]]; j < G::COL_PTR[G::VT_COLS[i] + 1]; ++j)
-                if (G::COL_SLOT[j] >= 0 && G::RE_COL_REG[j] < 0) ++n;
+        for (int i = vt_col_ptr(w); i < vt_col_ptr(w + 1); ++i)
+            for (int j = G::COL_PTR[vt_cols(i)]; j < G::COL_PTR[vt_cols(i) + 1]; ++j)
+                if (G::COL_SLOT[j] >= 0 && col_reg_all(j) < 0) ++n;
         return n;
     }
     static constexpr int rot_share() {
@@ -55,18 +79,19 @@
         int left = RCAP;
         for (int w = 0; w < G::W; ++w) {
             const int a = col_slot_edges(w), b = col_slot_edges(WV);
-            if (a > b || (a == b && w < WV)) left -= G::RE_NROT[w];
-        }
-        return left < 0 ? 0 : (left < G::RE_NROT[WV] ? left : G::RE_NROT[WV]);
+            if (a > b || (a == b && w < WV)) left -= nrot(w);
+        }
+        return left < 0 ? 0 : (left < nrot(WV) ? left : nrot(WV));
     }
     static constexpr int NROT = rot_share();
-    static constexpr int row_rot(int e) { return REG && G::RE_ROW_ROT[e] < NROT ? G::RE_ROW_ROT[e] : -1; }
-    static constexpr int col_rot(int j) { return REG && G::RE_COL_ROT[j] < NROT ? G::RE_COL_ROT[j] : -1; }
-    static constexpr int C0 = G::VT_COL_PTR[WV], NC = G::VT_COL_PTR[WV + 1] - C0;
-    static constexpr int T0 = G::VT_PTR[WV], NT = G::VT_PTR[WV + 1] - T0;
+    static constexpr int row_rot(int e) { return REG && row_rot_all(e) < NROT ? row_rot_all(e) : -1; }
+    static constexpr int col_rot(int j) { return REG && col_rot_all(j) < NROT ? col_rot_all(j) : -1; }
+    static constexpr int C0 = vt_col_ptr(WV), NC = vt_col_ptr(WV + 1) - C0;
+    static constexpr int T0 = vt_ptr(WV), NT = vt_ptr(WV + 1) - T0;
+    static constexpr int col(int i) { return vt_cols(C0 + i); }
     static constexpr int col_index(int col) {
         for (int i = 0; i < NC; ++i)
-            if (G::VT_COLS[C0 + i] == col) return i;
+            if (vt_cols(C0 + i) == col) return i;
         return -1;
     }
     struct Tab {
@@ -86,7 +111,7 @@
             }
         };
         for (int i = 0; i < NC; ++i) {
-            const int c = G::VT_COLS[C0 + i];
+            const int c = vt_cols(C0 + i);
             const int dv = G::COL_PTR[c + 1] - G::COL_PTR[c];
             if (dv > t.maxdv) t.maxdv = dv;
             for (int j = G::COL_PTR[c]; j < G::COL_PTR[c + 1]; ++j)
@@ -199,12 +224,12 @@
 template <class G, int OUT>
 using DecOutFor = std::conditional_t<OUT < 0, NoOut, DecOut<G, OUT>>;
 
-template <class G, int ALGO, int WV, bool BAIL, int CAP, int RCAP, bool REG>
+template <class G, int ALGO, int WV, bool BAIL, int CAP, int RCAP, bool REG, bool JOINT>
 struct FixedBody {
     static_assert(!BAIL || ALGO == LDPC_ALGO_MINSUM, "only min-sum has a fast and an exact check update");
     static constexpr bool kBail = BAIL;
     static constexpr bool kPeel = true;
-    using P = FxPlan<G, WV, CAP, RCAP, REG>;
+    using P = FxPlan<G, WV, CAP, RCAP, REG, JOINT>;
     static constexpr int ZM4 = 4 * G::Z - 1;
     static constexpr int NEXT = P::T.next > 0 ? P::T.next : 1;
     static constexpr int NCOL = P::NC > 0 ? P::NC : 1;
@@ -213,7 +238,7 @@
     static constexpr int NRG = P::NREG > 0 ? P::NREG : 1;
     static constexpr int NRT = P::NROT > 0 ? P::NROT : 1;
     float ext[NEXT];
-    float cllr[NCOL];
+    float cllr[NCOL + (JOINT ? 1 : 0)];
     uint32_t rot[NSH];
     float msg[NRG];
     float rmsg[NRT];
@@ -248,7 +273,7 @@
         });
         addtid_begin(C.lds);
         sfor<P::NC>([&](auto i) {
-            constexpr int I = decltype(i)::value, COL = G::VT_COLS[P::C0 + I];
+            constexpr int I = decltype(i)::value, COL = P::col(I);
             constexpr int P0 = G::COL_PTR[COL], DV = G::COL_PTR[COL + 1] - P0;
             cllr[I] = L.llr_at(COL * 4 * G::Z + L.k4);
             nan |= !(fabsf(cllr[I]) < INFINITY);
@@ -275,10 +300,12 @@
                 v[E] = msg[P::row_reg(P0 + E)];
             else if constexpr (P::row_rot(P0 + E) >= 0)
                 v[E] = rmsg[P::row_rot(P0 + E)];
-            else if constexpr (SL >= 0)
+            else if constexpr (SL >= 0) {
+                static_assert(P::T.shidx[P::inv_shift(P::row_shift(P0 + E))] >= 0, "rot[] holds the rotation");
                 v[E] = lds_rd_abs<SL * 256>(rot[P::T.shidx[P::inv_shift(P::row_shift(P0 + E))]]);
-            else
+            } else {
                 v[E] = ext[P::ext_index(I, E)];
+            }
         });
     }
 
@@ -399,12 +426,13 @@
     template <int TK>
     struct Task {
         static constexpr int X = P::T0 + TK;
-        static constexpr int CA = G::VT_A[X], CB = G::VT_B[X];
+        static constexpr int CA = P::vt_a(X), CB = P::vt_b(X);
         static constexpr int PA = G::COL_PTR[CA], DA = G::COL_PTR[CA + 1] - PA;
         static constexpr int PB = CB >= 0 ? G::COL_PTR[CB] : 0, DB = CB >= 0 ? G::COL_PTR[CB + 1] - PB : 0;
         static_assert(DB <= DA, "pair tasks: A is the longer column");
         static constexpr int IA = P::col_index(CA), IB = CB >= 0 ? P::col_index(CB) : 0;
         static constexpr int NMSG = DA + DB;
+        static_assert(IA >= 0 && IB >= 0, "a task's columns are columns of its wave");
     };
     struct TaskIn {
         f32x2 cp[MAXDV];
@@ -417,8 +445,10 @@
             return msg[P::col_reg(X)];
         else if constexpr (P::col_rot(X) >= 0)
             return rmsg[P::col_rot(X)];
-        else
+        else {
+            static_assert(P::T.shidx[P::col_shift(X)] >= 0, "rot[] holds the rotation");
             return lds_rd_abs<G::COL_SLOT[X] * 256>(rot[P::T.shidx[P::col_shift(X)]]);
+        }
     }
     template <int X>
     __device__ __forceinline__ void v2c_out(float o) {
@@ -592,7 +622,7 @@
     init_ctx(C, Tc, lds, alpha, out_dtype, bits);
     if constexpr (BAIL) C.redo = redo;
     fx_by_wave<G>(__builtin_amdgcn_readfirstlane((int)threadIdx.x >> 6), [&](auto wv) {
-        FixedBody<G, ALGO, decltype(wv)::value, BAIL, reg_edge_cap<ES, BAIL>(), rot_edge_cap<ES, BAIL>(), reg_edges(ALGO)> body;
+        FixedBody<G, ALGO, decltype(wv)::value, BAIL, reg_edge_cap<ES, BAIL>(), rot_edge_cap<ES, BAIL>(), reg_edges(ALGO), joint_family<G, ALGO, ES, BAIL>()> body;
         flood_drive<ES>(body, C, L, B, max_iter, O, W);
 #ifdef LDPC_TIMELINE
         if constexpr (ES == LDPC_ES_OFF) tl_bracket(O.timeline, decltype(wv)::value, t_in);
diff --git a/ldpc-neuralnetwork-decoder_amd/csrc/gen/fixed_codes.hpp b/ldpc-neuralnetwork-decoder_amd/csrc/gen/fixed_codes.hpp
--- a/ldpc-neuralnetwork-decoder_amd/csrc/gen/fixed_codes.hpp
+++ b/ldpc-neuralnetwork-decoder_amd/csrc/gen/fixed_codes.hpp
@@ -37,6 +37,25 @@
     static constexpr int RE_ROW_ROT[197] = {-1, -1, -1, -1, -1, -1, -1, -1, -1, 0, -1, 1, -1, -1, -1, -1, -1, -1, 0, -1, -1, -1, -1, -1, -1, -1, -1, 0, -1, -1, -1, 1, -1, -1, -1, -1, -1, -1, -1, -1, -1, -1, -1, -1, -1, -1, -1, -1, -1, -1, 2, -1, -1, -1, -1, -1, -1, -1, -1, -1, -1, -1, -1, -1, -1, -1, -1, -1, 0, -1, -1, -1, -1, -1, -1, -1, -1, -1, -1, -1, -1, -1, -1, -1, -1, -1, -1, -1, -1, -1, -1, -1, -1, -1, -1, -1, -1, -1, -1, -1, -1, -1, -1, -1, -1, -1, -1, -1, -1, -1, -1, -1, -1, -1, -1, -1, -1, -1, -1, -1, -1, -1, -1, -1, -1, -1, -1, -1, -1, -1, -1, -1, -1, -1, -1, 2, -1, -1, 3, -1, -1, -1, -1, -1, -1, -1, -1, 1, -1, -1, -1, -1, -1, -1, -1, -1, -1, -1, -1, -1, -1, -1, -1, -1, 4, -1, -1, 2, -1, -1, -1, -1, 3, -1, -1, -1, -1, -1, -1, -1, -1, -1, -1, -1, -1, -1, -1, 3, -1, -1, 5, -1, -1, -1, -1, -1, -1};
     static constexpr int RE_COL_ROT[197] = {-1, -1, 0, -1, -1, -1, -1, -1, -1, -1, -1, -1, -1, -1, -1, -1, -1, 1, -1, -1, -1, -1, -1, -1, -1, -1, -1, -1, -1, -1, 0, -1, -1, -1, -1, -1, -1, -1, -1, -1, -1, -1, -1, -1, -1, -1, 0, -1, -1, 2, -1, -1, -1, -1, -1, -1, 0, -1, -1, -1, -1, -1, -1, -1, -1, 1, -1, -1, -1, -1, -1, -1, -1, -1, -1, -1, -1, -1, -1, -1, -1, -1, -1, -1, -1, -1, -1, 1, -1, -1, -1, -1, -1, -1, -1, -1, -1, -1, -1, -1, -1, -1, -1, -1, -1, -1, -1, -1, -1, -1, -1, -1, -1, -1, -1, -1, -1, -1, -1, 4, -1, 5, -1, -1, -1, -1, 2, -1, -1, -1, -1, -1, -1, -1, -1, 3, -1, -1, -1, -1, -1, -1, -1, -1, -1, 2, 3, -1, -1, -1, -1, -1, -1, -1, 3, -1, -1, -1, -1, -1, -1, -1, -1, -1, -1, -1, -1, -1, -1, -1, -1, -1, -1, -1, -1, -1, -1, -1, -1, -1, -1, -1, -1, -1, -1, -1, -1, -1, -1, -1, -1, -1, -1, -1, -1, -1, -1};
     static constexpr int RE_NROT[4] = {4, 4, 1, 6};
+    static constexpr int RE_J_CAP = 24;
+    static constexpr int RE_J_RHO[42] = {3, 2, 0, 2, 1, 1, 0, 0, 2, 1, 3, 0, 1, 2, 1, 3, 0, 2, 0, 0, 2, 2, 1, 1, 0, 0, 2, 0, 1, 2, 0, 3, 2, 0, 1, 1, 2, 1, 1, 1, 0, 2};
+    static constexpr int RE_J_ROW_SHIFT[197] = {0, 0, 3, 1, 0, 0, 3, 3, 1, 0, 3, 3, 0, 2, 2, 2, 2, 2, 1, 2, 0, 0, 0, 1, 0, 0, 2, 0, 0, 2, 3, 0, 0, 2, 2, 2, 0, 3, 0, 1, 0, 2, 3, 0, 0, 1, 3, 0, 1, 0, 2, 0, 1, 3, 0, 3, 0, 0, 0, 0, 0, 2, 0, 2, 2, 0, 1, 2, 0, 3, 0, 3, 3, 0, 2, 0, 0, 0, 0, 3, 1, 1, 0, 0, 0, 2, 0, 2, 0, 1, 1, 2, 2, 0, 3, 3, 2, 0, 2, 0, 0, 2, 0, 2, 2, 0, 2, 2, 0, 3, 0, 1, 0, 0, 3, 3, 2, 2, 0, 0, 2, 3, 0, 1, 0, 0, 3, 1, 2, 3, 0, 0, 0, 0, 0, 3, 1, 2, 0, 2, 0, 3, 0, 3, 2, 0, 1, 0, 2, 2, 3, 0, 1, 0, 0, 1, 0, 3, 0, 2, 0, 2, 0, 0, 3, 0, 0, 2, 1, 1, 2, 1, 0, 1, 2, 0, 0, 2, 0, 0, 1, 0, 3, 3, 1, 0, 1, 3, 1, 0, 3, 0, 0, 3, 3, 0, 2};
+    static constexpr int RE_J_COL_SHIFT[197] = {0, 1, 1, 0, 0, 3, 0, 2, 3, 1, 2, 0, 3, 2, 0, 0, 0, 0, 0, 0, 2, 0, 0, 2, 2, 3, 2, 1, 0, 0, 0, 0, 0, 0, 3, 0, 0, 0, 3, 2, 3, 1, 2, 0, 3, 3, 0, 0, 3, 3, 2, 3, 0, 0, 0, 1, 0, 0, 0, 0, 3, 0, 0, 3, 2, 3, 2, 3, 0, 3, 2, 3, 0, 0, 0, 2, 1, 3, 3, 0, 0, 3, 3, 2, 2, 3, 2, 0, 0, 1, 0, 0, 0, 2, 1, 1, 0, 0, 1, 2, 0, 0, 2, 0, 0, 0, 2, 2, 0, 2, 2, 0, 0, 3, 1, 2, 2, 2, 1, 3, 0, 3, 3, 2, 0, 0, 2, 3, 0, 3, 0, 0, 0, 0, 3, 0, 3, 0, 2, 0, 0, 2, 2, 2, 0, 2, 3, 0, 2, 0, 0, 0, 1, 0, 0, 0, 1, 0, 0, 1, 1, 0, 0, 2, 1, 3, 0, 1, 2, 1, 3, 0, 2, 0, 0, 2, 2, 1, 1, 0, 0, 2, 0, 1, 2, 0, 3, 2, 0, 1, 1, 2, 1, 1, 1, 0, 2};
+    static constexpr int RE_J_ROW_REG[197] = {0, -1, -1, -1, 1, -1, -1, -1, -1, 2, -1, -1, 3, -1, -1, -1, -1, -1, -1, -1, -1, 0, 1, -1, -1, 2, -1, 3, 4, -1, -1, -1, 5, -1, -1, -1, -1, -1, 0, -1, -1, -1, -1, 0, -1, -1, -1, 1, -1, 2, -1, -1, -1, -1, 3, -1, -1, -1, 4, -1, 5, -1, 1, -1, -1, 2, -1, -1, -1, -1, 4, -1, -1, 5, -1, -1, -1, 3, -1, -1, -1, -1, -1, 6, 7, -1, 4, -1, 5, -1, -1, -1, -1, 6, -1, -1, -1, 7, -1, -1, 8, -1, 9, -1, -1, 6, -1, -1, -1, -1, 10, -1, -1, 11, -1, -1, -1, -1, 8, 9, -1, -1, 10, -1, 7, 8, -1, -1, -1, -1, 6, -1, 9, -1, -1, -1, -1, -1, 11, -1, 10, -1, -1, -1, -1, 7, -1, 11, -1, -1, -1, 8, -1, 9, -1, -1, 12, -1, 12, -1, 13, -1, 13, -1, -1, -1, 14, -1, -1, -1, -1, -1, 12, -1, -1, -1, 10, -1, 14, 15, -1, 13, -1, -1, -1, 15, -1, -1, -1, 16, -1, 17, -1, -1, -1, 14, -1};
+    static constexpr int RE_J_COL_REG[197] = {0, -1, -1, -1, -1, -1, 4, -1, -1, -1, -1, 6, -1, -1, 7, 9, 10, 11, 12, 14, -1, 15, -1, -1, -1, -1, -1, -1, -1, 1, -1, 3, -1, 4, -1, 8, 10, 11, -1, -1, -1, -1, -1, 13, -1, -1, 3, 10, -1, -1, -1, -1, 13, -1, 16, -1, 2, -1, -1, 8, -1, 0, 4, -1, -1, -1, -1, -1, 1, -1, -1, -1, -1, 7, 8, -1, -1, -1, -1, 1, 3, -1, -1, -1, -1, -1, -1, -1, 0, -1, 3, 4, 5, -1, -1, -1, -1, 10, -1, -1, 1, 5, -1, 6, 8, -1, -1, -1, 2, -1, -1, 6, 9, -1, -1, -1, -1, -1, -1, -1, 14, -1, -1, -1, 0, -1, -1, -1, 2, -1, 5, 6, 7, 9, -1, 12, -1, 14, -1, -1, 5, -1, -1, -1, 13, -1, -1, 2, -1, -1, -1, 7, -1, 9, 11, 12, -1, 15, 17, -1, -1, -1, -1, -1, -1, -1, -1, -1, -1, -1, -1, -1, -1, -1, -1, -1, -1, -1, -1, -1, -1, -1, -1, -1, -1, -1, -1, -1, -1, -1, -1, -1, -1, -1, -1, -1, -1};
+    static constexpr int RE_J_NREG[4] = {15, 18, 11, 16};
+    static constexpr int RE_J_CHK_PTR[5] = {0, 12, 22, 31, 42};
+    static constexpr int RE_J_CHK_ROWS[42] = {4, 9, 12, 14, 15, 16, 17, 19, 20, 35, 38, 41, 2, 3, 13, 21, 22, 26, 31, 33, 37, 40, 5, 6, 7, 10, 11, 24, 28, 30, 36, 0, 1, 8, 18, 23, 25, 27, 29, 32, 34, 39};
+    static constexpr int RE_J_ROW_ROT[197] = {-1, -1, -1, 0, -1, -1, -1, -1, 1, -1, -1, -1, -1, -1, -1, -1, -1, 2, -1, -1, -1, -1, -1, 0, -1, -1, -1, -1, -1, -1, -1, -1, -1, -1, 1, 2, -1, 0, -1, -1, -1, -1, 0, -1, -1, -1, -1, -1, 1, -1, -1, -1, -1, 2, -1, -1, -1, -1, -1, -1, -1, -1, -1, -1, -1, -1, -1, -1, -1, -1, -1, -1, -1, -1, 3, -1, -1, -1, -1, 1, -1, -1, -1, -1, -1, -1, -1, -1, -1, -1, -1, -1, -1, -1, -1, 2, -1, -1, -1, -1, -1, -1, -1, -1, -1, -1, 3, -1, -1, -1, -1, -1, -1, -1, -1, 3, -1, -1, -1, -1, -1, -1, -1, -1, -1, -1, -1, -1, -1, -1, -1, -1, -1, -1, -1, 3, -1, -1, -1, -1, -1, 4, -1, -1, -1, -1, -1, -1, -1, -1, -1, -1, 4, -1, -1, -1, -1, -1, -1, -1, -1, -1, -1, -1, 4, -1, -1, 5, -1, -1, 4, -1, -1, -1, -1, -1, -1, -1, -1, -1, -1, -1, -1, 5, -1, -1, -1, 6, -1, -1, 5, -1, -1, 6, -1, -1, -1};
+    static constexpr int RE_J_COL_ROT[197] = {-1, 1, -1, -1, -1, -1, -1, -1, -1, -1, -1, -1, -1, -1, -1, -1, -1, -1, -1, -1, -1, -1, -1, -1, -1, 0, -1, -1, -1, -1, -1, -1, -1, -1, 2, -1, -1, -1, -1, -1, -1, -1, 4, -1, 6, -1, -1, -1, -1, 3, -1, -1, -1, -1, -1, 0, -1, -1, -1, -1, -1, -1, -1, -1, -1, -1, -1, 0, -1, 2, -1, -1, -1, -1, -1, -1, -1, -1, -1, -1, -1, -1, -1, -1, 3, 4, -1, -1, -1, 1, -1, -1, -1, -1, -1, 4, -1, -1, -1, -1, -1, -1, -1, -1, -1, -1, -1, -1, -1, 3, -1, -1, -1, -1, 0, 1, -1, -1, -1, 4, -1, 5, -1, -1, -1, -1, -1, -1, -1, 1, -1, -1, -1, -1, 3, -1, 5, -1, 2, -1, -1, -1, -1, -1, -1, 5, 6, -1, 2, -1, -1, -1, -1, -1, -1, -1, -1, -1, -1, -1, -1, -1, -1, -1, -1, -1, -1, -1, -1, -1, -1, -1, -1, -1, -1, -1, -1, -1, -1, -1, -1, -1, -1, -1, -1, -1, -1, -1, -1, -1, -1, -1, -1, -1, -1, -1, -1};
+    static constexpr int RE_J_NROT[4] = {7, 6, 5, 7};
+    static constexpr int RE_J_VT_COL_PTR[5] = {0, 2, 7, 10, 14};
+    static constexpr int RE_J_VT_COLS[14] = {1, 11, 2, 4, 8, 10, 13, 5, 7, 9, 0, 3, 6, 12};
+    static constexpr int RE_J_VT_PTR[5] = {0, 2, 5, 7, 10};
+    static constexpr int RE_J_VT_A[10] = {1, 11, 4, 10, 13, 5, 9, 0, 3, 12};
+    static constexpr int RE_J_VT_B[10] = {-1, -1, -1, 8, 2, 7, -1, -1, -1, 6};
+    static constexpr int RE_J_OPS_CHK[4] = {43, 40, 45, 45};
+    static constexpr int RE_J_OPS_VAR[4] = {41, 42, 43, 47};
 };
 
 struct BG2_Z32 {
@@ -73,6 +92,25 @@
     static constexpr int RE_ROW_ROT[197] = {-1, -1, -1, -1, -1, 0, -1, 1, 0, -1, 1, -1, -1, -1, -1, -1, -1, -1, -1, -1, -1, -1, 0, -1, -1, -1, -1, 0, -1, -1, -1, 1, -1, -1, -1, -1, -1, -1, -1, -1, -1, -1, -1, -1, -1, -1, -1, -1, -1, -1, -1, -1, -1, -1, -1, -1, -1, -1, -1, -1, -1, -1, -1, 1, -1, -1, -1, -1, -1, -1, -1, -1, -1, -1, -1, -1, -1, -1, -1, -1, -1, -1, -1, -1, -1, -1, -1, 2, -1, -1, -1, -1, -1, -1, -1, -1, -1, 2, -1, -1, -1, -1, -1, -1, -1, -1, -1, -1, -1, -1, -1, -1, -1, -1, -1, -1, -1, -1, -1, -1, -1, -1, -1, -1, -1, -1, 3, -1, -1, -1, -1, -1, -1, -1, -1, -1, -1, -1, -1, -1, -1, -1, -1, -1, -1, -1, -1, 2, -1, -1, -1, 4, -1, -1, -1, -1, -1, -1, -1, -1, -1, -1, -1, -1, 2, -1, 3, -1, -1, -1, -1, -1, -1, -1, -1, -1, -1, -1, -1, 3, -1, -1, -1, 5, -1, -1, -1, -1, -1, -1, 4, 5, -1, -1, 6, -1, -1};
     static constexpr int RE_COL_ROT[197] = {-1, 0, -1, -1, -1, -1, -1, -1, -1, -1, -1, -1, -1, -1, -1, -1, -1, 2, -1, 3, -1, -1, -1, -1, -1, -1, -1, -1, -1, -1, -1, -1, -1, -1, -1, -1, -1, -1, -1, -1, -1, -1, -1, -1, -1, -1, 0, -1, -1, -1, -1, -1, -1, -1, -1, -1, -1, -1, -1, -1, 1, -1, -1, -1, -1, -1, -1, -1, -1, -1, -1, 3, -1, -1, 4, -1, -1, -1, 6, -1, -1, -1, -1, 2, -1, -1, -1, 1, -1, -1, -1, -1, -1, -1, -1, -1, -1, -1, -1, -1, 0, -1, 1, -1, -1, 0, -1, -1, -1, -1, -1, -1, -1, -1, -1, -1, -1, -1, -1, 2, -1, 4, 1, -1, -1, -1, -1, -1, -1, -1, -1, -1, 2, -1, -1, -1, 5, -1, -1, -1, -1, -1, -1, -1, -1, -1, -1, -1, -1, -1, -1, -1, -1, -1, -1, -1, -1, 3, 5, -1, -1, -1, -1, -1, -1, -1, -1, -1, -1, -1, -1, -1, -1, -1, -1, -1, -1, -1, -1, -1, -1, -1, -1, -1, -1, -1, -1, -1, -1, -1, -1, -1, -1, -1, -1, -1, -1};
     static constexpr int RE_NROT[4] = {4, 7, 3, 6};
+    static constexpr int RE_J_CAP = 24;
+    static constexpr int RE_J_RHO[42] = {0, 0, 0, 0, 25, 25, 4, 13, 18, 3, 0, 8, 17, 13, 13, 11, 24, 4, 30, 7, 6, 20, 1, 18, 21, 28, 3, 9, 30, 4, 12, 22, 14, 28, 11, 1, 6, 5, 26, 17, 0, 10};
+    static constexpr int RE_J_ROW_SHIFT[197] = {9, 21, 12, 26, 29, 13, 0, 0, 7, 6, 29, 29, 2, 28, 0, 28, 0, 0, 17, 18, 12, 20, 16, 1, 0, 0, 8, 26, 30, 8, 17, 22, 18, 0, 0, 0, 12, 15, 0, 25, 0, 2, 27, 24, 0, 25, 31, 8, 17, 0, 2, 4, 14, 0, 25, 16, 1, 13, 0, 16, 24, 18, 14, 16, 0, 26, 3, 11, 25, 0, 21, 0, 19, 20, 26, 0, 8, 16, 0, 31, 17, 0, 15, 19, 11, 13, 0, 30, 16, 21, 13, 30, 26, 0, 11, 3, 6, 0, 10, 24, 2, 0, 22, 4, 4, 26, 0, 16, 30, 30, 27, 0, 7, 0, 15, 3, 6, 0, 30, 6, 20, 31, 0, 1, 9, 29, 0, 18, 3, 0, 29, 21, 0, 24, 28, 0, 18, 3, 29, 3, 17, 0, 9, 0, 3, 5, 30, 22, 0, 4, 19, 28, 21, 0, 12, 0, 23, 22, 0, 26, 20, 14, 0, 0, 7, 28, 30, 0, 15, 11, 26, 9, 0, 1, 18, 12, 0, 6, 0, 28, 5, 25, 28, 0, 26, 0, 29, 19, 17, 0, 11, 24, 0, 11, 15, 0, 10};
+    static constexpr int RE_J_COL_SHIFT[197] = {9, 7, 17, 12, 0, 31, 0, 11, 19, 0, 30, 26, 30, 0, 9, 0, 17, 22, 0, 30, 18, 0, 21, 18, 8, 15, 2, 14, 16, 14, 25, 16, 15, 0, 3, 2, 27, 0, 31, 3, 0, 0, 26, 25, 11, 12, 26, 0, 0, 0, 3, 19, 0, 12, 0, 26, 6, 12, 0, 29, 29, 20, 30, 15, 0, 29, 8, 27, 8, 0, 0, 0, 24, 5, 28, 26, 9, 28, 15, 29, 2, 17, 0, 30, 0, 0, 28, 22, 24, 17, 25, 21, 20, 16, 18, 21, 0, 0, 29, 0, 16, 18, 16, 19, 30, 13, 28, 0, 0, 26, 6, 29, 0, 0, 1, 0, 0, 26, 0, 7, 0, 11, 0, 0, 0, 0, 2, 16, 26, 31, 16, 0, 0, 22, 3, 0, 0, 0, 0, 0, 24, 10, 4, 3, 20, 0, 19, 0, 0, 1, 0, 11, 21, 6, 29, 23, 15, 28, 24, 25, 25, 4, 13, 18, 3, 0, 8, 17, 13, 13, 11, 24, 4, 30, 7, 6, 20, 1, 18, 21, 28, 3, 9, 30, 4, 12, 22, 14, 28, 11, 1, 6, 5, 26, 17, 0, 10};
+    static constexpr int RE_J_ROW_REG[197] = {-1, -1, -1, -1, -1, -1, 0, -1, -1, -1, -1, -1, -1, -1, 0, -1, -1, 1, -1, -1, -1, -1, -1, -1, 2, -1, -1, -1, -1, -1, -1, -1, -1, 0, -1, 1, -1, -1, 0, -1, -1, -1, -1, -1, 1, -1, -1, -1, -1, 2, -1, -1, -1, 2, -1, -1, -1, -1, 3, -1, -1, -1, -1, -1, 1, -1, -1, -1, -1, 2, -1, -1, -1, -1, -1, 3, -1, -1, 3, -1, -1, 4, -1, -1, -1, -1, 3, -1, -1, -1, -1, -1, -1, 4, -1, -1, -1, 5, -1, -1, -1, 6, -1, -1, -1, -1, 4, -1, -1, -1, -1, 5, -1, 6, -1, -1, -1, 5, -1, -1, -1, -1, 4, -1, -1, -1, 7, -1, -1, 5, -1, -1, 6, -1, -1, 6, -1, -1, -1, -1, -1, 7, -1, 8, -1, -1, -1, -1, 7, -1, -1, -1, -1, 7, -1, 9, -1, -1, 8, -1, -1, -1, 8, 9, -1, -1, -1, 9, -1, -1, -1, -1, 8, -1, -1, -1, 10, -1, 10, -1, -1, -1, -1, 9, -1, 10, -1, -1, -1, 11, -1, -1, -1, -1, -1, 10, -1};
+    static constexpr int RE_J_COL_REG[197] = {-1, -1, -1, -1, -1, -1, 3, -1, -1, 4, -1, -1, -1, 5, -1, 6, -1, -1, 8, -1, -1, 10, -1, -1, -1, -1, -1, -1, -1, -1, -1, -1, -1, 3, -1, -1, -1, 6, -1, -1, 8, 9, -1, -1, -1, -1, -1, 4, 5, 6, -1, -1, 8, -1, 11, -1, -1, -1, 3, -1, -1, -1, -1, -1, 7, -1, -1, -1, -1, 2, 6, 7, -1, -1, -1, -1, -1, -1, -1, -1, -1, -1, 2, -1, 4, 7, -1, -1, -1, -1, -1, -1, -1, -1, -1, -1, 9, 10, -1, 0, -1, -1, -1, -1, -1, -1, -1, 0, 2, -1, -1, -1, 7, 0, -1, -1, 1, -1, 5, -1, 10, -1, -1, -1, 0, 1, -1, -1, -1, -1, -1, 4, 5, -1, -1, 8, 9, 10, 1, 2, -1, -1, -1, -1, -1, 9, -1, -1, 1, -1, 3, -1, -1, -1, -1, -1, -1, -1, -1, -1, -1, -1, -1, -1, -1, -1, -1, -1, -1, -1, -1, -1, -1, -1, -1, -1, -1, -1, -1, -1, -1, -1, -1, -1, -1, -1, -1, -1, -1, -1, -1, -1, -1, -1, -1, -1, -1};
+    static constexpr int RE_J_NREG[4] = {12, 11, 11, 11};
+    static constexpr int RE_J_CHK_PTR[5] = {0, 10, 20, 31, 42};
+    static constexpr int RE_J_CHK_ROWS[42] = {3, 6, 11, 22, 24, 26, 30, 33, 36, 40, 1, 2, 8, 13, 21, 25, 29, 32, 34, 39, 0, 9, 10, 14, 18, 19, 20, 27, 28, 31, 37, 4, 5, 7, 12, 15, 16, 17, 23, 35, 38, 41};
+    static constexpr int RE_J_ROW_ROT[197] = {-1, 0, -1, -1, 1, -1, -1, -1, 0, -1, 1, -1, -1, -1, -1, -1, -1, -1, 2, -1, -1, 3, 4, -1, -1, -1, -1, 0, -1, -1, -1, 1, -1, -1, -1, -1, -1, -1, -1, -1, -1, -1, 0, -1, -1, -1, -1, -1, 2, -1, -1, -1, -1, -1, -1, 1, -1, -1, -1, -1, 5, -1, 2, -1, -1, -1, -1, -1, 3, -1, -1, -1, -1, 3, 4, -1, -1, -1, -1, 2, -1, -1, -1, 6, -1, -1, -1, 4, -1, -1, -1, -1, -1, -1, -1, -1, -1, -1, -1, -1, -1, -1, 3, -1, -1, -1, -1, -1, -1, -1, 5, -1, -1, -1, -1, -1, -1, -1, 7, -1, -1, -1, -1, -1, -1, 4, -1, -1, -1, -1, 5, -1, -1, -1, -1, -1, 6, -1, 7, -1, -1, -1, -1, -1, -1, -1, -1, 8, -1, -1, 8, -1, 9, -1, -1, -1, -1, -1, -1, -1, 9, -1, -1, -1, -1, -1, 10, -1, -1, -1, -1, 5, -1, -1, -1, 10, -1, -1, -1, -1, -1, -1, 6, -1, -1, -1, -1, 11, -1, -1, -1, 11, -1, -1, 7, -1, -1};
+    static constexpr int RE_J_COL_ROT[197] = {-1, 0, 2, -1, -1, -1, -1, -1, -1, -1, -1, -1, -1, -1, -1, -1, -1, 8, -1, 10, -1, -1, 0, -1, -1, -1, -1, -1, -1, 2, 3, -1, -1, -1, -1, -1, 5, -1, -1, -1, -1, -1, -1, -1, -1, -1, 0, -1, -1, -1, -1, 8, -1, 10, -1, -1, -1, -1, -1, 4, 1, 3, -1, -1, -1, -1, -1, 0, -1, -1, -1, -1, -1, -1, -1, -1, 5, 6, 7, 1, -1, -1, -1, 4, -1, -1, -1, 1, -1, 2, -1, -1, 3, -1, 6, 9, -1, -1, -1, -1, 4, -1, -1, 6, 7, -1, -1, -1, -1, 4, -1, 5, -1, -1, -1, -1, -1, -1, -1, -1, -1, -1, -1, -1, -1, -1, -1, 1, -1, 2, -1, -1, -1, 3, -1, -1, -1, -1, -1, -1, 5, -1, -1, -1, 9, -1, 11, -1, -1, -1, -1, -1, -1, -1, 7, -1, -1, -1, 11, -1, -1, -1, -1, -1, -1, -1, -1, -1, -1, -1, -1, -1, -1, -1, -1, -1, -1, -1, -1, -1, -1, -1, -1, -1, -1, -1, -1, -1, -1, -1, -1, -1, -1, -1, -1, -1, -1};
+    static constexpr int RE_J_NROT[4] = {12, 12, 6, 8};
+    static constexpr int RE_J_VT_COL_PTR[5] = {0, 4, 8, 11, 14};
+    static constexpr int RE_J_VT_COLS[14] = {2, 7, 9, 13, 0, 4, 8, 12, 1, 6, 10, 3, 5, 11};
+    static constexpr int RE_J_VT_PTR[5] = {0, 2, 5, 7, 9};
+    static constexpr int RE_J_VT_A[9] = {2, 7, 0, 4, 12, 1, 10, 3, 11};
+    static constexpr int RE_J_VT_B[9] = {9, 13, -1, -1, 8, -1, 6, -1, 5};
+    static constexpr int RE_J_OPS_CHK[4] = {46, 48, 48, 48};
+    static constexpr int RE_J_OPS_VAR[4] = {50, 50, 50, 40};
 };
 
 }
```

New measurement: 77.50 million, median of 6. +2.0%, better.
